# Li-Jinjie/ndp_nmpc_qd

Hardware: AMD Instinct MI355X
Metric: NMPC solves/sec (N=20, 1 RTI iter + downwash MLP) at batch (higher is better)
Workload: dtype f64

## Files before the change

ndp_nmpc_qd_amd/batched.py:

```python
import ctypes as C

import numpy as np

from . import _lib
from .params import downwash_params as DP
from .params import nmpc_params as CP


class NdpError(RuntimeError):
    pass


class BatchedNMPC:
    def __init__(self, batch, N=CP.N_node, disturbance=False, n_rti=1, qp_mode=_lib.QP_AUTO, device=0,
                 dt=CP.th_pred, load_mlp=None, **cfg_overrides):
        self._lib = _lib.load()
        if "ipm_refine" not in cfg_overrides and (7 * int(N) - 3 > 192 or cfg_overrides.get("qp_precision", 0)):
            cfg_overrides = dict(cfg_overrides, ipm_refine=0)
        self.cfg = _lib.default_cfg(batch=int(batch), N=int(N), n_rti=int(n_rti), use_fd=int(bool(disturbance)),
                                    qp_mode=int(qp_mode), device=int(device), dt=float(dt), r_horiz=DP.r_horiz,
                                    **cfg_overrides)
        self.B, self.N = int(batch), int(N)
        self.disturbance = bool(disturbance)
        self._h = C.c_void_p()
        rc = self._lib.ndp_create(C.byref(self.cfg), C.byref(self._h))
        if rc != 0:
            self._h = None
            raise NdpError(f"ndp_create failed ({rc}): {self._lib.ndp_last_error(None).decode()}")
        if load_mlp is None:
            load_mlp = self.disturbance
        if load_mlp:
            self.set_mlp_weights(_lib.load_weights())

    def close(self):
        if getattr(self, "_h", None):
            self._lib.ndp_destroy(self._h)
            self._h = None

    def __del__(self):
        try:
            self.close()
        except Exception:
            pass

    def _check(self, rc, what):
        if rc < 0:
            raise NdpError(f"{what} failed ({rc}): {self._lib.ndp_last_error(self._h).decode()}")
        return rc

    def set_mlp_weights(self, blob):
        blob = np.ascontiguousarray(blob, dtype=np.float32)
        self._check(self._lib.ndp_set_mlp_weights(self._h, _lib.ptr(blob), blob.size), "ndp_set_mlp_weights")
        self._mlp_installed = None

    def reset(self, xr, ur):
        xr = _lib.f64(xr, (self.B, self.N + 1, 10))
        ur = _lib.f64(ur, (self.B, self.N, 4))
        self._check(self._lib.ndp_reset(self._h, _lib.ptr(xr), _lib.ptr(ur)), "ndp_reset")

    def update(self, x0, xr, ur, f=None, other=None, ego_xy=None, raise_on_status=True, full=False):
        x0 = _lib.f64(x0, (self.B, 10))
        xr = _lib.f64(xr, (self.B, self.N + 1, 10))
        ur = _lib.f64(ur, (self.B, self.N, 4))
        u0 = np.empty((self.B, 4), dtype=np.float64)
        if f is not None and other is None and np.asarray(f).dtype == np.float64:
            f64 = _lib.f64(f, (self.B, self.N + 1, 3))
            X = U = st = it = None
            if full:
                X, U = np.empty((self.B, self.N + 1, 10)), np.empty((self.B, self.N, 4))
                st, it = np.empty(self.B, dtype=np.int32), np.empty(self.B, dtype=np.int32)
            rc = self._check(self._lib.ndp_step_ex_f64(self._h, _lib.ptr(x0), _lib.ptr(xr), _lib.ptr(ur), _lib.ptr(f64), _lib.ptr(u0),
                                                       _lib.ptr(X), _lib.ptr(U), _lib.ptr(st), _lib.ptr(it)), "ndp_step_ex_f64")
            if rc != 0 and raise_on_status:
                raise Exception("acados acados_ocp_solver returned status {}. Exiting.".format(rc))
            return (u0, X, U, st, it) if full else u0
        f32 = None if f is None else np.ascontiguousarray(f, dtype=np.float32).reshape(self.B, self.N + 1, 3)
        other = _lib.f64(other, (self.B, self.N + 1, 10))
        ego_xy = _lib.f64(ego_xy, (self.B, 2))
        if full:
            X, U = np.empty((self.B, self.N + 1, 10)), np.empty((self.B, self.N, 4))
            st, it = np.empty(self.B, dtype=np.int32), np.empty(self.B, dtype=np.int32)
            rc = self._check(self._lib.ndp_step_ex(self._h, _lib.ptr(x0), _lib.ptr(xr), _lib.ptr(ur), _lib.ptr(f32),
                                                   _lib.ptr(other), _lib.ptr(ego_xy), _lib.ptr(u0), _lib.ptr(X), _lib.ptr(U),
                                                   _lib.ptr(st), _lib.ptr(it)), "ndp_step_ex")
        else:
            rc = self._check(self._lib.ndp_step(self._h, _lib.ptr(x0), _lib.ptr(xr), _lib.ptr(ur), _lib.ptr(f32),
                                                _lib.ptr(other), _lib.ptr(ego_xy), _lib.ptr(u0)), "ndp_step")
        if rc != 0 and raise_on_status:
            raise Exception("acados acados_ocp_solver returned status {}. Exiting.".format(rc))
        return (u0, X, U, st, it) if full else u0

    def update_begin(self, x0, xr, ur, f=None, other=None, ego_xy=None, want_iterate=False):
        x0 = _lib.f64(x0, (self.B, 10))
        xr = _lib.f64(xr, (self.B, self.N + 1, 10))
        ur = _lib.f64(ur, (self.B, self.N, 4))
        f32 = None if f is None else np.ascontiguousarray(f, dtype=np.float32).reshape(self.B, self.N + 1, 3)
        other = _lib.f64(other, (self.B, self.N + 1, 10))
        ego_xy = _lib.f64(ego_xy, (self.B, 2))
        self._check(self._lib.ndp_step_begin(self._h, _lib.ptr(x0), _lib.ptr(xr), _lib.ptr(ur), _lib.ptr(f32), _lib.ptr(other),
                                             _lib.ptr(ego_xy), 1 if want_iterate else 0), "ndp_step_begin")

    def update_end(self, raise_on_status=True, full=False, out=None):
        u0 = np.empty((self.B, 4), dtype=np.float64) if out is None else out
        st = it = X = U = None
        if full:
            X, U = np.empty((self.B, self.N + 1, 10)), np.empty((self.B, self.N, 4))
            st, it = np.empty(self.B, dtype=np.int32), np.empty(self.B, dtype=np.int32)
        rc = self._check(self._lib.ndp_step_end(self._h, _lib.ptr(u0), _lib.ptr(X), _lib.ptr(U), _lib.ptr(st), _lib.ptr(it)),
                         "ndp_step_end")
        if rc != 0 and raise_on_status:
            raise Exception("acados acados_ocp_solver returned status {}. Exiting.".format(rc))
        return (u0, X, U, st, it) if full else u0

    def update_debug(self, x0, xr, ur, f=None, other=None, ego_xy=None):
        x0, xr, ur = _lib.f64(x0, (1, 10)), _lib.f64(xr, (1, self.N + 1, 10)), _lib.f64(ur, (1, self.N, 4))
        f32 = None if f is None else np.ascontiguousarray(f, dtype=np.float32).reshape(1, self.N + 1, 3)
        other, ego_xy = _lib.f64(other, (1, self.N + 1, 10)), _lib.f64(ego_xy, (1, 2))
        u0 = np.empty((1, 4))
        dump = np.zeros(self._lib.ndp_debug_lds_doubles(self.N))
        self._check(self._lib.ndp_step_debug(self._h, _lib.ptr(x0), _lib.ptr(xr), _lib.ptr(ur), _lib.ptr(f32),
                                             _lib.ptr(other), _lib.ptr(ego_xy), _lib.ptr(u0), _lib.ptr(dump)),
                    "ndp_step_debug")
        return u0, dump

    def downwash(self, other, ego_ref, ego_xy=None):
        other = _lib.f64(other, (self.B, self.N + 1, 10))
        ego_ref = _lib.f64(ego_ref, (self.B, self.N + 1, 10))
        ego_xy = _lib.f64(ego_xy, (self.B, 2))
        f = np.empty((self.B, self.N + 1, 3), dtype=np.float32)
        self._check(self._lib.ndp_downwash(self._h, _lib.ptr(other), _lib.ptr(ego_ref), _lib.ptr(ego_xy), _lib.ptr(f)),
                    "ndp_downwash")
        return f

    def throttle_reset(self):
        self._check(self._lib.ndp_throttle_reset(self._h), "ndp_throttle_reset")

    def throttle_update(self, vz, throttle):
        vz, throttle = _lib.f64(vz, (self.B,)), _lib.f64(throttle, (self.B,))
        k = np.empty(self.B)
        self._check(self._lib.ndp_throttle_update(self._h, _lib.ptr(vz), _lib.ptr(throttle), _lib.ptr(k)), "ndp_throttle_update")
        return k

    def throttle_state(self):
        st = np.empty((self.B, 8))
        self._check(self._lib.ndp_throttle_get_state(self._h, _lib.ptr(st)), "ndp_throttle_get_state")
        return st

    def actuator_cmd(self, u0, k_throttle):
        u0, k = _lib.f64(u0, (self.B, 4)), _lib.f64(k_throttle, (self.B,))
        cmd = np.empty((self.B, 4))
        self._check(self._lib.ndp_actuator_cmd(self._h, _lib.ptr(u0), _lib.ptr(k), _lib.ptr(cmd)), "ndp_actuator_cmd")
        return cmd

    def relay_reset(self):
        self._check(self._lib.ndp_relay_reset(self._h), "ndp_relay_reset")

    def relay_formation(self, form):
        form = _lib.f64(form, (self.B, 3))
        off = np.empty((self.B, 3))
        self._check(self._lib.ndp_relay_formation(self._h, _lib.ptr(form), _lib.ptr(off)), "ndp_relay_formation")
        return off

    def relay_reference(self, xr_lead):
        xr_lead = _lib.f64(xr_lead, (self.B, self.N + 1, 10))
        out = np.empty_like(xr_lead)
        self._check(self._lib.ndp_relay_reference(self._h, _lib.ptr(xr_lead), _lib.ptr(out)), "ndp_relay_reference")
        return out

    def ref_set_trajectory(self, coeff_x, coeff_y, coeff_z, coeff_yaw, time_cum, time_seg, final_pt):
        time_seg = _lib.f64(time_seg)
        n_seg = time_seg.shape[1]
        cx, cy, cz = (_lib.f64(np.reshape(c, (self.B, n_seg * 8)), (self.B, n_seg * 8)) for c in (coeff_x, coeff_y, coeff_z))
        cyaw = _lib.f64(np.reshape(coeff_yaw, (self.B, n_seg * 4)), (self.B, n_seg * 4))
        time_cum, final_pt = _lib.f64(time_cum, (self.B, n_seg + 1)), _lib.f64(final_pt, (self.B, 3))
        self._check(self._lib.ndp_ref_set_trajectory(self._h, n_seg, _lib.ptr(cx), _lib.ptr(cy), _lib.ptr(cz), _lib.ptr(cyaw),
                                                     _lib.ptr(time_cum), _lib.ptr(_lib.f64(time_seg, (self.B, n_seg))),
                                                     _lib.ptr(final_pt)), "ndp_ref_set_trajectory")

    def ref_window(self, t):
        t = _lib.f64(t, (self.B,))
        xr, ur = np.empty((self.B, self.N + 1, 10)), np.empty((self.B, self.N, 4))
        self._check(self._lib.ndp_ref_window(self._h, _lib.ptr(t), _lib.ptr(xr), _lib.ptr(ur)), "ndp_ref_window")
        return xr, ur

    def ref_list_reset(self):
        self._check(self._lib.ndp_ref_list_reset(self._h), "ndp_ref_list_reset")

    def ref_list_fix_pt(self, x_odom, quirk_b1=True):
        x_odom = _lib.f64(x_odom, (self.B, 10))
        self._check(self._lib.ndp_ref_list_fix_pt(self._h, _lib.ptr(x_odom), int(bool(quirk_b1))), "ndp_ref_list_fix_pt")

    def ref_list_window(self, t=None):
        t = _lib.f64(t, (self.B,))
        xr, ur = np.empty((self.B, self.N + 1, 10)), np.empty((self.B, self.N, 4))
        self._check(self._lib.ndp_ref_list_window(self._h, _lib.ptr(t), _lib.ptr(xr), _lib.ptr(ur)), "ndp_ref_list_window")
        return xr, ur

    def ref_list_advance_device(self, t, stream=None):
        import torch
        self._check(self._lib.ndp_ref_list_advance_device(self._h, self._dptr(t, torch.float64, (self.B,)), self._stream(stream)),
                    "ndp_ref_list_advance_device")

    def ref_list_window_device(self, xr_out, ur_out, stream=None):
        import torch
        self._check(self._lib.ndp_ref_list_window_device(
            self._h, self._dptr(xr_out, torch.float64, (self.B, self.N + 1, 10)),
            self._dptr(ur_out, torch.float64, (self.B, self.N, 4)), self._stream(stream)), "ndp_ref_list_window_device")

    def ref_window_device(self, t, xr_out, ur_out, stream=None):
        import torch
        self._check(self._lib.ndp_ref_window_device(
            self._h, self._dptr(t, torch.float64, (self.B,)), self._dptr(xr_out, torch.float64, (self.B, self.N + 1, 10)),
            self._dptr(ur_out, torch.float64, (self.B, self.N, 4)), self._stream(stream)), "ndp_ref_window_device")

    def tick_config(self, other_index=None, gate=True):
        oi = None if other_index is None else np.ascontiguousarray(other_index, dtype=np.int32).reshape(self.B)
        self._check(self._lib.ndp_tick_config(self._h, _lib.ptr(oi), 1 if gate else 0), "ndp_tick_config")

    def tick_reset(self):
        self._check(self._lib.ndp_tick_reset(self._h), "ndp_tick_reset")

    def _tick_in(self, x_odom, t, vz, throttle, estimate, want_u0):
        flags = (_lib.TICK_ESTIMATE if estimate else 0) | (_lib.TICK_WANT_U0 if want_u0 else 0)
        if t is not None and np.ndim(t) == 0:
            t, flags = np.array([float(t)]), flags | _lib.TICK_T_UNIFORM
        else:
            t = _lib.f64(t, (self.B,))
        return (_lib.f64(x_odom, (self.B, 10)), t, _lib.f64(vz, (self.B,)), _lib.f64(throttle, (self.B,)), flags)

    def tick_begin(self, x_odom, t=None, vz=None, throttle=None, estimate=False, want_u0=False):
        x, t, vz, th, flags = self._tick_in(x_odom, t, vz, throttle, estimate, want_u0)
        self._check(self._lib.ndp_tick_begin(self._h, _lib.ptr(x), _lib.ptr(t), _lib.ptr(vz), _lib.ptr(th), flags), "ndp_tick_begin")

    def tick_end(self, raise_on_status=True, full=False, out=None):
        cmd = np.empty((self.B, 4)) if out is None else out
        u0 = st = it = None
        if full:
            u0, st, it = np.empty((self.B, 4)), np.empty(self.B, dtype=np.int32), np.empty(self.B, dtype=np.int32)
        rc = self._check(self._lib.ndp_tick_end(self._h, _lib.ptr(cmd), _lib.ptr(u0), _lib.ptr(st), _lib.ptr(it)), "ndp_tick_end")
        if rc != 0 and raise_on_status:
            raise Exception("acados acados_ocp_solver returned status {}. Exiting.".format(rc))
        return (cmd, u0, st, it) if full else cmd

    def tick(self, x_odom, t=None, vz=None, throttle=None, estimate=False, raise_on_status=True, full=False):
        x, t, vz, th, flags = self._tick_in(x_odom, t, vz, throttle, estimate, full)
        cmd = np.empty((self.B, 4))
        u0 = st = it = None
        if full:
            u0, st, it = np.empty((self.B, 4)), np.empty(self.B, dtype=np.int32), np.empty(self.B, dtype=np.int32)
        rc = self._check(self._lib.ndp_tick(self._h, _lib.ptr(x), _lib.ptr(t), _lib.ptr(vz), _lib.ptr(th), flags, _lib.ptr(cmd),
                                            _lib.ptr(u0), _lib.ptr(st), _lib.ptr(it)), "ndp_tick")
        if rc != 0 and raise_on_status:
            raise Exception("acados acados_ocp_solver returned status {}. Exiting.".format(rc))
        return (cmd, u0, st, it) if full else cmd

    def tick_device(self, x_odom, cmd_out, t=None, vz=None, throttle=None, estimate=False, u0_out=None, stream=None):
        import torch
        B = self.B
        flags = _lib.TICK_ESTIMATE if estimate else 0
        if t is not None and not isinstance(t, torch.Tensor):
            t_host = np.array([float(t)])
            tp, flags = _lib.ptr(t_host), flags | _lib.TICK_T_UNIFORM
        else:
            tp = self._dptr(t, torch.float64, (B,))
        self._check(self._lib.ndp_tick_device(
            self._h, self._dptr(x_odom, torch.float64, (B, 10)), tp,
            self._dptr(vz, torch.float64, (B,)), self._dptr(throttle, torch.float64, (B,)), flags,
            self._dptr(cmd_out, torch.float64, (B, 4)), self._dptr(u0_out, torch.float64, (B, 4)), self._stream(stream)),
            "ndp_tick_device")

    def tick_config_remote(self, windows, other_index, gate=True):
        import torch
        assert isinstance(windows, torch.Tensor) and windows.is_cuda and windows.is_contiguous() and windows.dtype == torch.float64
        assert windows.dim() == 3 and windows.shape[1] == self.N + 1 and windows.shape[2] in (6, 10)
        oi = np.ascontiguousarray(other_index, dtype=np.int32).reshape(self.B)
        self._tick_windows = windows
# ... 552 lines not shown
```

ndp_nmpc_qd_amd/csrc/host.hpp:

```cpp
#pragma once
#include <hip/hip_runtime.h>

#include <atomic>
#include <cstdint>
#include <memory>
#include <mutex>
#include <string>
#include <vector>

#include "wave_gfx950.hpp"
#include "cfg_params.hpp"
#include "kern_args.hpp"
#include "rti_table.hpp"

#define NDP_HIDDEN __attribute__((visibility("hidden")))

using namespace ndp;

struct ndp_handle {
    ndp_cfg cfg;
    RtiParams P;
    int lds_per_wave = 0;
    int waves = 4;
    int n_simd = 1024;
    mutable std::atomic<uint64_t> rti_launched{0};
    bool use_queue = false;
    bool queue_auto = false;
    unsigned long long *hIpm = nullptr;
    unsigned long long ipm_seen = 0, steps_seen = 0;
    unsigned queue_launches = 0;
    hipStream_t stream = nullptr;
    double *dX = nullptr, *dU = nullptr;
    float *dForce = nullptr, *dFrag = nullptr;
    double *dKC = nullptr;
    int *dTables = nullptr;
    signed char *dAct = nullptr;
    int sens_level = 0;
    double *dSensU0 = nullptr, *dSensU = nullptr, *dSensX = nullptr;
    double *dPSensXr = nullptr, *dPSensUr = nullptr, *dPSensF = nullptr;
    double *dVjp = nullptr;
    int *dVjpSt = nullptr;
    signed char *dVjpAct = nullptr;
    float *dFragT = nullptr, *dGwPart = nullptr;
    double *dThr = nullptr;
    double *dStamps = nullptr;
    double *dTraj = nullptr;
    int traj_seg = 0;
    double *dRingX = nullptr, *dRingU = nullptr;
    unsigned long long list_n = 0;
    int segc_par = 0;
    int list_step = 5;
    int *dTickIndex = nullptr;
    double *dTickThrust = nullptr;
    bool tick_gate = true;
    const double *tick_remote = nullptr;
    int tick_remote_stride = 6;
    struct TickSlot { bool busy = false, want_u0 = false; } tslot[2];
    double *dRelay = nullptr;
    double *sThr = nullptr;
    float *dForceAB[2] = {nullptr, nullptr};
    unsigned long long *dProto = nullptr;
    hipStream_t aux = nullptr;
    hipEvent_t evFork = nullptr, evJoin = nullptr;
    unsigned prefetch_timeout_us = 100000, pf_groups_rti = 1, pf_ntiles = 1;
    unsigned *dQctr = nullptr;
    int *dQids = nullptr;
    bool have_mlp = false;
    unsigned char *dIn = nullptr, *dOut = nullptr;
    size_t off_x0 = 0, off_xr = 0, off_ur = 0, off_f = 0, off_other = 0, off_ego = 0, in_bytes = 0;
    size_t off_u0 = 0, off_st = 0, off_it = 0, out_bytes = 0, out_all = 0;
    double *sx0 = nullptr, *sxr = nullptr, *sur = nullptr, *sother = nullptr, *sego = nullptr, *su0 = nullptr, *sdbg = nullptr;
    float *sf = nullptr;
    int *dStatus = nullptr, *dIters = nullptr;
    const int *lastStatus = nullptr, *lastIters = nullptr;
    struct HostSlot {
        unsigned char *hIn = nullptr, *hOut = nullptr;
        hipEvent_t evOut = nullptr;
        bool busy = false, want_iter = false;
        double *dump = nullptr;
    } slot[2];
    bool slots_ready = false;
    bool track_steps = false;
    bool last_step_tracked = false;
    bool track_pending = false;
    hipEvent_t stepDone[4] = {nullptr, nullptr, nullptr, nullptr};
    unsigned step_seq = 0;
    double host_us[4] = {0, 0, 0, 0};
    int host_cores = 0, pack_threads = 0;
    int slot_head = 0, slot_tail = 0, slots_busy = 0;
    std::unique_ptr<struct PackPool> pool;
    hipEvent_t evLast = nullptr;
    bool ev_pending = false;
    int timing = 0;
    int64_t launch_no[2] = {0, 0};
    bool timing_open = false;
    struct Ev { hipEvent_t a, b; int kind; };
    std::vector<Ev> events;
    std::mutex mu;
    std::string err;
};

#define NDP_HIP(h, call)                                                                   \
    do {                                                                                   \
        hipError_t e_ = (call);                                                            \
        if (e_ != hipSuccess) {                                                            \
            (h)->err = std::string(#call) + ": " + hipGetErrorString(e_);                  \
            return -(int)e_ - 1000;                                                        \
        }                                                                                  \
    } while (0)

static inline RingGeom ring_geom(const ndp_handle *h) { return RingGeom{h->list_step, h->cfg.N + 1}; }

enum { FRT_TOTAL = 2 * 128 * 64 };
enum { VJ_MAX_GROUPS = 256 };
static inline int mlp_vjp_groups(const ndp_handle *h)
{
    const int ntiles = (h->cfg.batch * (h->cfg.N + 1) + 31) / 32, ngroups = (ntiles + 3) / 4;
    return ngroups < VJ_MAX_GROUPS ? ngroups : VJ_MAX_GROUPS;
}

enum { TICK_ESTIMATE = NDP_TICK_ESTIMATE, TICK_WANT_U0 = NDP_TICK_WANT_U0, TICK_T_UNIFORM = NDP_TICK_T_UNIFORM };

static inline size_t nxs(const ndp_handle *h) { return (size_t)h->cfg.batch * (h->cfg.N + 1) * NX; }
static inline size_t nus(const ndp_handle *h) { return (size_t)h->cfg.batch * h->cfg.N * NU; }
static inline size_t nfs(const ndp_handle *h) { return (size_t)h->cfg.batch * (h->cfg.N + 1) * 3; }
static inline size_t up256(size_t n) { return (n + 255) & ~(size_t)255; }
static inline size_t act_bytes(const ndp_handle *h) { return (size_t)h->cfg.batch * (size_t)act_pitch(h->cfg.N); }
struct TrajView {
    double *coeff, *tcum, *tseg, *fpt, *segc[2];
    int *hint;
    size_t doubles;
};
static inline TrajView traj_view(double *base, size_t B, size_t S)
{
    TrajView v;
    size_t o = 0;
    auto part = [&](size_t n) { double *p = base ? base + o : nullptr; o += n; return p; };
    v.coeff = part(B * S * 28); v.tcum = part(B * (S + 1)); v.tseg = part(B * S); v.fpt = part(B * 3);
    v.segc[0] = part(B * SEGC_PER); v.hint = reinterpret_cast<int *>(part((B * 4 + 7) / 8)); v.segc[1] = part(B * SEGC_PER);
    v.doubles = o;
    return v;
}
static inline TrajView traj_view(const ndp_handle *h) { return traj_view(h->dTraj, (size_t)h->cfg.batch, (size_t)h->traj_seg); }
static inline void copy_ipm_iters(int32_t *dst, const int32_t *src, size_t n)
{
    for (size_t i = 0; i < n; ++i) dst[i] = src[i] & ITERS_IPM_MASK;
}

struct Neigh {
    const double *other = nullptr;
    int stride = NX;
    const int *index = nullptr;
    const double *ego_xy = nullptr;
    size_t pitch = 0;
    size_t ego_pitch = 0;
};

struct StepOut {
    int *status = nullptr;
    int *iters = nullptr;
    double *Xm = nullptr, *Um = nullptr;
    hipEvent_t done = nullptr;
    size_t xr_pitch = 0, ur_pitch = 0;
    double *cmd = nullptr;
    const double *kthr = nullptr;
    double *thrust_keep = nullptr;
    bool f_f64 = false;
    const TickArgs *tick = nullptr;
};

enum RecomputeId { RC_WVJP, RC_JVP, RC_VJP };

extern "C" {
NDP_HIDDEN bool queue_shape(const ndp_handle *h);
NDP_HIDDEN void launch_kern(const ndp_handle *h, RtiId id, hipStream_t s, KernArgs &ka, SensArgs &sa, hipEvent_t start = nullptr,
                            hipEvent_t stop = nullptr);
NDP_HIDDEN const void *recompute_kernel(RecomputeId id, bool n20);
NDP_HIDDEN hipError_t rti_set_lds(bool sens, int lds_bytes, const char **what);
NDP_HIDDEN hipError_t mlp_prepare(void);
NDP_HIDDEN int launch_mlp(ndp_handle *h, const Neigh &nb, const double *d_ego, float *d_f, hipStream_t s, size_t ego_pitch = 0);
NDP_HIDDEN void launch_tick_pre(const TickPre &a, hipStream_t s);
NDP_HIDDEN int sens_refuse(ndp_handle *h, const char *what);
NDP_HIDDEN int note_stream(ndp_handle *h, hipStream_t s);
NDP_HIDDEN int set_device(ndp_handle *h);
NDP_HIDDEN int wait_all(ndp_handle *h);
NDP_HIDDEN int begin_timing(ndp_handle *h, hipStream_t s, int kind, bool defer = false);
NDP_HIDDEN int end_timing(ndp_handle *h, hipStream_t s);
NDP_HIDDEN bool can_fuse(const ndp_handle *h);
NDP_HIDDEN int launch_rti(ndp_handle *h, const double *d_x0, const double *d_xr, const double *d_ur, const float *d_f, double *d_u0,
                          double *d_dbg, hipStream_t s, const Neigh *nb = nullptr, const StepOut *so = nullptr, bool prefetched = false);
NDP_HIDDEN int enqueue_step(ndp_handle *h, const double *d_x0, const double *d_xr, const double *d_ur, const float *d_f, const Neigh &nb,
                            double *d_u0, double *d_dbg, hipStream_t s, const StepOut *so = nullptr);
NDP_HIDDEN int ensure_slots(ndp_handle *h);
NDP_HIDDEN int launch_plant_force(ndp_handle *h, const double *d_x, const int *d_index, int gate, double scale, double *d_f, double *d_xy,
                                  hipStream_t s);
NDP_HIDDEN hipError_t mlp_multi_prepare(void);
NDP_HIDDEN int check_neigh(ndp_handle *h, const char *who, int K);
NDP_HIDDEN int launch_mlp_multi(ndp_handle *h, const double *d_other, int other_stride, const int *d_index, int K, const double *d_ego,
                                const double *d_ego_xy, float *d_f, hipStream_t s);
NDP_HIDDEN int launch_plant_force_multi(ndp_handle *h, const double *d_x, const int *d_index, int K, int gate, double scale, double *d_f,
                                        double *d_xy, hipStream_t s);
NDP_HIDDEN ThrCfg thr_cfg(const ndp_handle *h);
NDP_HIDDEN RefCfg ref_cfg(const ndp_handle *h, double toff);
NDP_HIDDEN void launch_throttle_reset(const ndp_handle *h);
NDP_HIDDEN int launch_list_window(ndp_handle *h, double *d_xr, double *d_ur, hipStream_t s);
NDP_HIDDEN int ensure_tick(ndp_handle *h);
NDP_HIDDEN int tick_step_enqueue(ndp_handle *h, hipStream_t s, const double *x_odom, double *cmd, double *u0, const double *windows,
                                 unsigned long long pos);
NDP_HIDDEN void make_fragments_t(const float *blob, float *frt);
NDP_HIDDEN hipError_t mlp_vjp_prepare(void);
NDP_HIDDEN int peer_mapped(const void *p);
NDP_HIDDEN void launch_pack_pv_list(const double *base, size_t pitch, int np1, double *pv, size_t B, hipStream_t s);
}
NDP_HIDDEN TickPre tick_pre(const ndp_handle *h, bool adv, const double *t, double t_all, bool est, const double *x_odom, const double *vz,
                            const double *throttle, double *pv = nullptr);

struct Entry {
    ndp_handle *h;
    std::unique_lock<std::mutex> lk;
    hipStream_t s = nullptr;
    int rc = -1;
    Entry(ndp_handle *h_, bool args, void *stream = nullptr, const char *refuse = nullptr) : h(h_)
    {
        if (!h) return;
// ... 15 lines not shown
```

ndp_nmpc_qd_amd/csrc/ndp_hip.hip:

```cpp
#include <hip/hip_runtime.h>
#include <hip/hip_ext.h>

#include <sched.h>
#include <stdio.h>

#include <atomic>
#include <chrono>
#include <condition_variable>
#include <cstdlib>
#include <cstring>
#include <memory>
#include <mutex>
#include <new>
#include <string>
#include <thread>
#include <type_traits>
#include <vector>

#include "host.hpp"
#include "cond_qp.hpp"
#include "mlp_tile.hpp"

namespace ndp {

// ... 154 lines not shown
    for (auto &e : h->events) { (void)hipEventDestroy(e.a); (void)hipEventDestroy(e.b); }
    if (h->evLast) (void)hipEventDestroy(h->evLast);
    if (h->aux) { (void)hipStreamSynchronize(h->aux); (void)hipStreamDestroy(h->aux); }
    for (hipEvent_t e : {h->evFork, h->evJoin, h->stepDone[0], h->stepDone[1], h->stepDone[2], h->stepDone[3]})
        if (e) (void)hipEventDestroy(e);
    h->pool.reset();
    void *ptrs[] = {h->dForceAB[0], h->dForceAB[1], h->dProto, h->dRingX, h->dTraj, h->dTables, h->dStamps, h->dRelay, h->dThr, h->sThr, h->dKC, h->dForce, h->dFrag,
                    h->dIn, h->dOut, h->sdbg, h->dQctr, h->dQids, h->dTickIndex, h->dTickThrust, h->dAct,
                    h->dSensU0, h->dSensU, h->dSensX, h->dPSensXr, h->dPSensUr, h->dPSensF, h->dVjp, h->dVjpSt, h->dVjpAct, h->dFragT, h->dGwPart};
    for (void *p : ptrs)
        if (p) (void)hipFree(p);
    for (auto &sl : h->slot) {
        if (sl.hIn) (void)hipHostFree(sl.hIn);
        if (sl.hOut) (void)hipHostFree(sl.hOut);
        if (sl.evOut) (void)hipEventDestroy(sl.evOut);
    }
    if (h->hIpm) {
        (void)hipDeviceSynchronize();
        (void)hipHostFree(h->hIpm);
    }
    if (h->stream) (void)hipStreamDestroy(h->stream);
    delete h;
    return 0;
}

static bool as_gamma_holds(const ndp_cfg &c, const double *Rd)
{
    if (c.as_iter_max <= 0) return true;
    double rd = 0.0;
    for (int i = 0; i < 4; ++i) rd = std::max(rd, std::fabs(c.dt * Rd[i]));
    return std::isfinite(c.as_gamma) && c.as_gamma >= NDP_AS_GAMMA_FLOOR * rd;
}

int ndp_create(const ndp_cfg *cfg, ndp_handle **out)
{
    if (!cfg || !out) { g_create_err = "ndp_create: null argument"; return -1; }
    *out = nullptr;
    if (cfg->batch < 1 || cfg->N < 2 || slots_for(cfg->N) > 5 || cfg->n_rti < 1 || cfg->qp_precision < 0 || cfg->qp_precision > 6 ||
        cfg->work_queue < 0 || cfg->work_queue > 2 || !(cfg->ts_nmpc > 0.0) || cfg->dt < cfg->ts_nmpc) {
        g_create_err = "ndp_create: need batch >= 1, 2 <= N <= 46, n_rti >= 1, qp_precision in 0..6, work_queue in 0..2, 0 < ts_nmpc <= dt";
        return -2;
    }
    if (cfg->qp_precision >= 5 && (cfg->N % 4 != 0 || cfg->N > 40)) {
        g_create_err = "ndp_create: the condensed study (qp_precision 5 / 6) tiles the 4N x 4N Hessian by 16: N must be a multiple of 4, at most 40";
        return -2;
    }
    if (!as_gamma_holds(*cfg, cfg->Rd)) {
        g_create_err = "ndp_create: as_gamma must be finite and at least 1e8 * max(dt * Rd) when as_iter_max > 0 (a weaker pin does not hold "
                       "its input on the bound)";
        return -2;
    }
    if (cfg->ipm_refine > 0 && (slots_for(cfg->N) > 3 || cfg->qp_precision != 0)) {
        g_create_err = "ndp_create: ipm_refine > 0 is not served for this shape: the refinement path (stiff sweeps + second solves while a STATE bound's "
                       "barrier term exceeds refine_gamma) lives in the three-slot fp64 kernels only (N <= 27, qp_precision 0); the five-slot kernels "
                       "(N >= 28) sit at the register limit without it.  Set ipm_refine = 0: strongly active state bounds at a tight tolerance then "
                       "end in status 4 (never a silent answer)";
        return -2;
    }
    {
        const double ratio = cfg->dt / cfg->ts_nmpc, nearest = (double)(long long)(ratio + 0.5);
        if (ratio - nearest > 1e-9 || nearest - ratio > 1e-9) {
            g_create_err = "ndp_create: dt must be a whole multiple of ts_nmpc (node spacing = every k-th entry of the reference list)";
            return -2;
        }
    }
    int ndev = 0;
    hipError_t e = hipGetDeviceCount(&ndev);
    if (e != hipSuccess || ndev <= cfg->device) {
        g_create_err = std::string("ndp_create: no usable HIP device (") + hipGetErrorString(e) + ")";
        return -3;
    }
    ndp_handle *h = new (std::nothrow) ndp_handle;
    if (!h) return -4;
    h->cfg = *cfg;
    h->P = to_params(*cfg);
    h->list_step = (int)(cfg->dt / cfg->ts_nmpc + 0.5);
    h->lds_per_wave = (lds_doubles(cfg->N) + 1) & ~1;
    if (cfg->qp_precision >= 5) h->lds_per_wave += (cond_extra_doubles(cfg->N) + 1) & ~1;
    const size_t per_wave_bytes = (size_t)h->lds_per_wave * sizeof(double);
    h->waves = 4;
    while (h->waves > 1 && per_wave_bytes * h->waves > 160 * 1024) h->waves >>= 1;
    if (const char *e = getenv("NDP_DEV_WAVES")) {
        const int w = atoi(e);
        if ((w == 1 || w == 2 || w == 4) && w <= h->waves) h->waves = w;
    }
    auto fail = [&](const char *what, hipError_t err) {
        g_create_err = std::string("ndp_create: ") + what + ": " + hipGetErrorString(err);
        ndp_destroy(h);
        return -5;
    };
    if ((e = hipSetDevice(cfg->device)) != hipSuccess) return fail("hipSetDevice", e);
    {
        hipDeviceProp_t prop;
        if ((e = hipGetDeviceProperties(&prop, cfg->device)) != hipSuccess) return fail("hipGetDeviceProperties", e);
        h->n_simd = 4 * prop.multiProcessorCount;
    }
    if (cfg->work_queue == 1 && !(queue_shape(h) && cfg->qp_mode == NDP_QP_AUTO)) {
        g_create_err = "ndp_create: work_queue = 1 needs qp_mode AUTO, qp_precision 0 and (N, n_rti) = (20, 1) or (40, 2)";
        delete h;
        return -2;
    }
    h->queue_auto = cfg->work_queue == 0 && queue_shape(h) && cfg->qp_mode == NDP_QP_AUTO && cfg->N == 20 && cfg->batch >= 2 * h->n_simd;
    h->use_queue = cfg->work_queue == 1 || (cfg->work_queue == 0 && queue_shape(h) && cfg->qp_mode == NDP_QP_AUTO && cfg->N == 40);
    if (h->queue_auto) {
        if ((e = hipHostMalloc((void **)&h->hIpm, 64, hipHostMallocDefault)) != hipSuccess) return fail("hipHostMalloc (work-list counter)", e);
        h->hIpm[0] = h->hIpm[1] = 0;
    }
    if ((e = hipStreamCreateWithFlags(&h->stream, hipStreamNonBlocking)) != hipSuccess) return fail("hipStreamCreate", e);
    if ((e = hipEventCreateWithFlags(&h->evLast, hipEventDisableTiming)) != hipSuccess) return fail("hipEventCreate", e);
    const size_t B = cfg->batch;
#define ALLOC(p, n)                                                                      \
    if ((e = hipMalloc((void **)&(p), (n))) != hipSuccess) return fail("hipMalloc " #p, e)
    ALLOC(h->dForce, nfs(h) * 4); ALLOC(h->dFrag, FR_TOTAL * 4); ALLOC(h->dFragT, FRT_TOTAL * 4); ALLOC(h->dGwPart, (size_t)mlp_vjp_groups(h) * NDP_MLP_NPARAM * 4); ALLOC(h->dKC, KC_HOST * 8);
    ALLOC(h->dThr, B * 8 * 8); ALLOC(h->sThr, B * 11 * 8);
    ALLOC(h->dRelay, B * 4 * 8);
    ALLOC(h->dQctr, 256); ALLOC(h->dQids, B * 4);
    ALLOC(h->dAct, B * (size_t)act_pitch(cfg->N));
    (void)hipMemsetAsync(h->dAct, 0, B * (size_t)act_pitch(cfg->N), h->stream);
    (void)hipMemsetAsync(h->dRelay, 0, B * 4 * 8, h->stream);
    (void)hipMemsetAsync(h->dQctr, 0, 256, h->stream);
    {
        double kc[KC_HOST];
        fill_kc(h->P, kc);
        if ((e = hipMemcpyAsync(h->dKC, kc, sizeof(kc), hipMemcpyHostToDevice, h->stream)) != hipSuccess) return fail("hipMemcpy kc", e);
        ALLOC(h->dTables, TB_WORDS * 4);
        std::vector<int> tb(TB_WORDS);
        fill_tables(cfg->N, tb.data(), (cfg->qp_precision == 3 || cfg->qp_precision == 4) ? 1 : 0);
        if ((e = hipMemcpyAsync(h->dTables, tb.data(), TB_WORDS * 4, hipMemcpyHostToDevice, h->stream)) != hipSuccess) return fail("hipMemcpy tables", e);
        if ((e = hipStreamSynchronize(h->stream)) != hipSuccess) return fail("hipStreamSynchronize", e);
    }
    {
        size_t o = 0;
        h->off_x0 = o; o += up256(B * NX * 8);
        h->off_xr = o; o += up256(nxs(h) * 8);
        h->off_ur = o; o += up256(nus(h) * 8);
        h->off_f = o; o += up256(nfs(h) * 8);
        h->off_other = o; o += up256(nxs(h) * 8);
        h->off_ego = o; o += up256(B * 2 * 8);
        h->in_bytes = o;
        o = 0;
        h->off_u0 = o; o += up256(B * NU * 8);
        h->off_st = o; o += up256(B * 4);
        h->off_it = o; o += up256(B * 4);
        h->out_bytes = o;
        h->out_all = h->out_bytes + (nxs(h) + nus(h)) * 8;
        ALLOC(h->dIn, h->in_bytes);
        ALLOC(h->dOut, h->out_all);
        h->dX = (double *)(h->dOut + h->out_bytes); h->dU = h->dX + nxs(h);
        h->sx0 = (double *)(h->dIn + h->off_x0); h->sxr = (double *)(h->dIn + h->off_xr); h->sur = (double *)(h->dIn + h->off_ur);
        h->sf = (float *)(h->dIn + h->off_f); h->sother = (double *)(h->dIn + h->off_other); h->sego = (double *)(h->dIn + h->off_ego);
        h->su0 = (double *)(h->dOut + h->off_u0); h->dStatus = (int *)(h->dOut + h->off_st); h->dIters = (int *)(h->dOut + h->off_it);
        h->lastStatus = h->dStatus; h->lastIters = h->dIters;
        ALLOC(h->sdbg, (size_t)(lds_doubles(cfg->N) + DBG_EXTRA) * 8);
    }
#undef ALLOC
    (void)hipMemsetAsync(h->dX, 0, nxs(h) * 8, h->stream);
    (void)hipMemsetAsync(h->dU, 0, nus(h) * 8, h->stream);
    (void)hipMemsetAsync(h->dOut, 0, h->out_bytes, h->stream);
    (void)hipMemsetAsync(h->dForce, 0, nfs(h) * 4, h->stream);
    const int lds_bytes = (int)(per_wave_bytes * h->waves);
    if ((e = mlp_prepare()) != hipSuccess) return fail("hipFuncSetAttribute(mlp_kernel)", e);
    if ((e = mlp_vjp_prepare()) != hipSuccess) return fail("hipFuncSetAttribute(mlp_vjp_kernel)", e);
    if ((e = mlp_multi_prepare()) != hipSuccess) return fail("hipFuncSetAttribute(mlp_multi_kernel)", e);
    const char *what = nullptr;
    if ((e = rti_set_lds(false, lds_bytes, &what)) != hipSuccess) return fail(what, e);
    launch_throttle_reset(h);
    if ((e = hipStreamSynchronize(h->stream)) != hipSuccess) return fail("hipStreamSynchronize", e);
    *out = h;
    return 0;
}

int begin_timing(ndp_handle *h, hipStream_t s, int kind, bool defer)
{
    h->timing_open = false;
    if (!h->timing || (h->launch_no[kind]++ % h->timing) != 0) return 0;
    h->timing_open = true;
    ndp_handle::Ev ev; ev.kind = kind;
    NDP_HIP(h, hipEventCreate(&ev.a)); NDP_HIP(h, hipEventCreate(&ev.b));
    if (!defer) NDP_HIP(h, hipEventRecord(ev.a, s));
    h->events.push_back(ev);
    return 0;
}
int end_timing(ndp_handle *h, hipStream_t s)
{
    if (!h->timing_open) return 0;
    NDP_HIP(h, hipEventRecord(h->events.back().b, s));
    return 0;
}

int note_stream(ndp_handle *h, hipStream_t s)
{
    if (s == h->stream) return 0;
    hipStreamCaptureStatus cs = hipStreamCaptureStatusNone;
    if (hipStreamIsCapturing(s, &cs) != hipSuccess || cs != hipStreamCaptureStatusNone) { (void)hipGetLastError(); return 0; }
    NDP_HIP(h, hipEventRecord(h->evLast, s));
    h->ev_pending = true;
    return 0;
}
int wait_all(ndp_handle *h)
{
    NDP_HIP(h, hipStreamSynchronize(h->stream));
    if (h->ev_pending) {
        NDP_HIP(h, hipEventSynchronize(h->evLast));
        h->ev_pending = false;
    }
    if (h->track_pending) {
        if (h->stepDone[h->step_seq & 3]) NDP_HIP(h, hipEventSynchronize(h->stepDone[h->step_seq & 3]));
        h->track_pending = false;
    }
    return 0;
}

int set_device(ndp_handle *h)
{
    NDP_HIP(h, hipSetDevice(h->cfg.device));
    return 0;
}

enum { QP_WINDOW = 8 };
static void queue_policy(ndp_handle *h, hipStream_t s)
{
    if (!h->queue_auto) return;
    const unsigned long long steps_now = ((volatile unsigned long long *)h->hIpm)[1], ipm_now = ((volatile unsigned long long *)h->hIpm)[0];
    if (steps_now >= h->steps_seen + QP_WINDOW && ipm_now >= h->ipm_seen) {
        const double frac = (double)(ipm_now - h->ipm_seen) / ((double)(steps_now - h->steps_seen) * (double)h->cfg.batch);
        if (frac >= 0.04) h->use_queue = true;
        else if (frac <= 0.015) h->use_queue = false;
        h->ipm_seen = ipm_now;
        h->steps_seen = steps_now;
    }
    if (++h->queue_launches < QP_WINDOW) return;
    h->queue_launches = 0;
    if (hipMemcpyAsync(h->hIpm, reinterpret_cast<unsigned long long *>(h->dQctr + 16), 16, hipMemcpyDeviceToHost, s) != hipSuccess) (void)hipGetLastError();
}

static RtiId rti_pick(const ndp_handle *h, bool fused, bool tick, bool prefetched, int phase)
{
    const int N = h->cfg.N, W = h->waves, pr = h->cfg.qp_precision, wi = W == 4 ? 0 : W == 2 ? 1 : 2;
    const bool ref = N == 20 && h->cfg.n_rti == 1;
    if (pr) {
        if (pr >= 3 && N == 40 && h->cfg.n_rti == 2 && W == 2) return pr == 3 ? K40_F32 : K40_BF16;
        return (RtiId)(KPREC1 + pr - 1);
    }
    if (h->sens_level > 0) {
        RtiId id;
        if (phase) id = phase == 2 ? S20_CONS : fused ? S20F_PROD : S20_PROD;
        else if (N == 20 && W == 4) id = fused ? S20F : S20;
        else if (W == 4) id = fused ? SF_4 : S_4;
        else id = fused ? SF_2 : S_2;
        if (!h->dPSensXr) return id;
        switch (id) {
        case S20F_PROD: return P20F_PROD;
        case S20_PROD: return P20_PROD;
        case S20_CONS: return P20_CONS;
        case S20F: return P20F;
        case S20: return P20;
        case SF_4: return PF_4;
        default: return PF_2;
        }
    }
    if (phase == 2) return N == 20 ? K20_CONS : K40_CONS;
    if (phase == 1) {
        if (N != 20) return K40_PROD;
        if (tick) return fused ? K20F_PROD_TICK : K20_PROD_TICK;
        return fused ? K20F_PROD : K20_PROD;
    }
    if (ref && W == 4) {
        if (tick) return fused ? K20F_TICK : K20_TICK;
        return fused ? K20F : prefetched ? K20_LATE : K20;
    }
    if (ref && W == 2) return fused ? K20F_W2 : K20_W2;
    if (N == 40 && h->cfg.n_rti == 2 && W == 2 && !fused) return K40;
    if (fused) return (RtiId)(K3F_4 + wi);
    return (RtiId)((slots_for(N) <= 3 ? K3_4 : K5_4) + wi);
}

int launch_rti(ndp_handle *h, const double *d_x0, const double *d_xr, const double *d_ur, const float *d_f,
               double *d_u0, double *d_dbg, hipStream_t s, const Neigh *nb, const StepOut *so, bool prefetched)
{
    int *d_status = so && so->status ? so->status : h->dStatus, *d_iters = so && so->iters ? so->iters : h->dIters;
    h->lastStatus = d_status; h->lastIters = d_iters;
    BatchPtrs bp{h->dKC, h->dTables, d_x0, d_xr, d_ur, d_f, h->dX, h->dU, d_u0, d_status, d_iters,
                 so ? so->Xm : nullptr, so ? so->Um : nullptr, d_dbg, h->dStamps,
                 so && so->xr_pitch ? so->xr_pitch : (size_t)(h->cfg.N + 1) * NX, so && so->ur_pitch ? so->ur_pitch : (size_t)h->cfg.N * NU, (size_t)NX,
                 so ? so->cmd : nullptr, so ? so->kthr : nullptr, so ? so->thrust_keep : nullptr, h->cfg.mass, so && so->f_f64 ? 1 : 0,
                 h->dAct};
    const bool fused = nb && nb->other;
    MlpArgs ma{fused ? h->dFrag : nullptr, fused ? nb->other : nullptr, fused ? nb->ego_xy : nullptr, h->dForce,
               h->cfg.r_horiz * h->cfg.r_horiz, fused ? nb->stride : NX, fused ? nb->index : nullptr, fused ? peer_mapped(nb->other) : 0,
               fused && nb->pitch ? nb->pitch : (size_t)(h->cfg.N + 1) * (fused ? nb->stride : NX), fused && nb->ego_pitch ? nb->ego_pitch : (size_t)2};
    QueueArgs qa{h->dQctr, h->dQids, reinterpret_cast<unsigned long long *>(h->dQctr + 16)};
    LateArgs la{prefetched ? h->dProto : nullptr, {h->dForceAB[0], h->dForceAB[1]}, h->prefetch_timeout_us,
                h->pf_groups_rti, h->pf_ntiles};
    KernArgs ka{h->P, bp, h->cfg.batch, h->lds_per_wave, ma, qa, la, so && so->tick ? *so->tick : TickArgs{}};
    SensArgs sa{h->dSensU0, h->sens_level >= 2 ? h->dSensU : nullptr, h->sens_level >= 2 ? h->dSensX : nullptr, h->sens_level};
    const bool tick1 = so && so->tick;
    const int pr = h->cfg.qp_precision;
    const bool q = h->use_queue && !d_dbg && !prefetched;
    h->last_step_tracked = false;
    if (h->track_steps) {
        hipStreamCaptureStatus cs = hipStreamCaptureStatusNone;
        if (hipStreamIsCapturing(s, &cs) != hipSuccess) { (void)hipGetLastError(); cs = hipStreamCaptureStatusNone; }
        if (cs != hipStreamCaptureStatusNone) {
            h->err = "tracked control steps (ndp_track_steps) cannot be launched on a stream that is being captured: switch tracking off "
                     "and order the exchange through the stream (ndp_xchg_begin's after_stream)";
            return -15;
        }
    }
    int rc = begin_timing(h, s, 0, true);
    if (rc) return rc;
    const bool ext_timing = h->timing_open && !q && !pr && !(so && so->done) && !h->track_steps;
    if (h->timing_open && !ext_timing) NDP_HIP(h, hipEventRecord(h->events.back().a, s));
    if (pr && fused) { h->err = "qp_precision != 0 supports f / no disturbance only (run ndp_downwash first)"; return -12; }
    hipEvent_t stop = nullptr;
    if (so && so->done) stop = so->done;
    else if (h->track_steps) { stop = h->stepDone[++h->step_seq & 3]; h->last_step_tracked = true; }
    if (h->sens_level > 0 && (prefetched || tick1)) { h->err = "launch_rti: the late-force and tick forms have no sensitivity kernel"; return -2; }
    launch_kern(h, rti_pick(h, fused, tick1, prefetched, q ? 1 : 0), s, ka, sa, ext_timing ? h->events.back().a : nullptr,
                ext_timing ? h->events.back().b : q || pr ? nullptr : stop);
    if (ext_timing) h->timing_open = false;
    NDP_HIP(h, hipGetLastError());
    if (q) {
        KernArgs kc = ka;
        kc.bp.f = fused ? h->dForce : d_f;
        kc.ma.frag = nullptr; kc.ma.other = nullptr;
        if (h->cfg.n_rti == 1 && h->cfg.as_iter_max <= 0) kc.P.qp_mode = QP_IPM_ALWAYS;
        launch_kern(h, rti_pick(h, fused, tick1, prefetched, 2), s, kc, sa);
        NDP_HIP(h, hipGetLastError());
        if (stop) hipExtLaunchKernelGGL(queue_reset_kernel, dim3(1), dim3(64), 0, s, nullptr, stop, 0, h->dQctr, qa.ipm_total);
        else hipLaunchKernelGGL(queue_reset_kernel, dim3(1), dim3(64), 0, s, h->dQctr, qa.ipm_total);
        NDP_HIP(h, hipGetLastError());
    } else if (pr && stop) NDP_HIP(h, hipEventRecord(stop, s));
    const int rce = end_timing(h, s);
    queue_policy(h, s);
    return rce;
}

bool can_fuse(const ndp_handle *h)
{
    return h->cfg.qp_precision == 0 && h->cfg.N + 1 <= 32 && slots_for(h->cfg.N) <= 3 &&
           (size_t)h->lds_per_wave * sizeof(double) * h->waves >= FR_TOTAL * sizeof(float);
}

int enqueue_step(ndp_handle *h, const double *d_x0, const double *d_xr, const double *d_ur, const float *d_f,
                 const Neigh &nb, double *d_u0, double *d_dbg, hipStream_t s, const StepOut *so)
{
    if (h->dPSensXr && !(nb.other && can_fuse(h)) && !(h->cfg.N == 20 && h->waves == 4)) {
        h->err = "ndp_step: parameter sensitivities at N != 20 (or 2 instances per workgroup) need the fused step (neighbour windows "
                 "given): the unfused kernel of a run-time horizon has none";
        return -2;
    }
    if ((d_f || nb.other) && !h->cfg.use_fd) { h->err = "ndp_step: a disturbance force needs use_fd = 1 (NDP model)"; return -8; }
    if (nb.other) {
        if (d_f) { h->err = "ndp_step: pass either f or other, not both"; return -7; }
        if (nb.stride != 10 && nb.stride != 6) { h->err = "ndp_step: other_stride must be 10 or 6"; return -13; }
        if (!h->have_mlp) { h->err = "downwash requested but ndp_set_mlp_weights was never called"; return -6; }
        if (can_fuse(h)) return launch_rti(h, d_x0, d_xr, d_ur, nullptr, d_u0, d_dbg, s, &nb, so);
        int rc = launch_mlp(h, nb, d_xr, h->dForce, s, so ? so->xr_pitch : 0);
        if (rc) return rc;
        d_f = h->dForce;
    }
    return launch_rti(h, d_x0, d_xr, d_ur, d_f, d_u0, d_dbg, s, nullptr, so);
}

int ndp_reset_device(ndp_handle *h, const void *d_xr, const void *d_ur, void *stream)
{
    Entry g(h, d_xr && d_ur, stream);
    if (g.rc) return g.rc;
    NDP_HIP(h, hipMemcpyAsync(h->dX, d_xr, nxs(h) * 8, hipMemcpyDefault, g.s));
    NDP_HIP(h, hipMemcpyAsync(h->dU, d_ur, nus(h) * 8, hipMemcpyDefault, g.s));
    NDP_HIP(h, hipMemsetAsync(h->dAct, 0, act_bytes(h), g.s));
    return g.noted(0);
}

int ndp_reset(ndp_handle *h, const double *xr, const double *ur)
{
    Entry g(h, xr && ur);
    if (g.rc) return g.rc;
    int rc = wait_all(h);
    if (rc) return rc;
    NDP_HIP(h, hipMemcpyAsync(h->dX, xr, nxs(h) * 8, hipMemcpyDefault, h->stream));
    NDP_HIP(h, hipMemcpyAsync(h->dU, ur, nus(h) * 8, hipMemcpyDefault, h->stream));
    NDP_HIP(h, hipMemsetAsync(h->dAct, 0, act_bytes(h), h->stream));
    return g.synced(0);
}

int ndp_step_device_ex(ndp_handle *h, const void *d_x0, const void *d_xr, const void *d_ur, const void *d_f,
                       const void *d_other, int other_stride, const void *d_other_index, const void *d_ego_xy,
                       void *d_u0, void *stream)
{
    Entry g(h, d_x0 && d_xr && d_ur && d_u0, stream);
    if (g.rc) return g.rc;
    Neigh nb;
    nb.other = (const double *)d_other; nb.stride = other_stride; nb.index = (const int *)d_other_index; nb.ego_xy = (const double *)d_ego_xy;
    return g.noted(enqueue_step(h, (const double *)d_x0, (const double *)d_xr, (const double *)d_ur, (const float *)d_f, nb,
                                (double *)d_u0, nullptr, g.s));
}

int ndp_step_device(ndp_handle *h, const void *d_x0, const void *d_xr, const void *d_ur, const void *d_f,
                    const void *d_other, const void *d_ego_xy, void *d_u0, void *stream)
{
    return ndp_step_device_ex(h, d_x0, d_xr, d_ur, d_f, d_other, NX, nullptr, d_ego_xy, d_u0, stream);
}

int ensure_slots(ndp_handle *h)
{
    if (h->slots_ready) return 0;
    for (int i = 0; i < 2; ++i) {
        ndp_handle::HostSlot &sl = h->slot[i];
        if (!sl.hIn) NDP_HIP(h, hipHostMalloc((void **)&sl.hIn, h->in_bytes, hipHostMallocDefault));
        if (!sl.hOut) {
            NDP_HIP(h, hipHostMalloc((void **)&sl.hOut, h->out_all, hipHostMallocDefault));
            memset(sl.hOut, 0, h->out_bytes);
        }
        if (!sl.evOut) NDP_HIP(h, hipEventCreateWithFlags(&sl.evOut, hipEventDisableTiming));
    }
    int nt = 0;
    h->host_cores = usable_cores();
    if (const char *e = getenv("NDP_PACK_THREADS")) nt = atoi(e);
    else if (h->in_bytes > 2 * PACK_CHUNK) nt = (h->host_cores / 2 > 8 ? 8 : h->host_cores / 2) - 1;
    h->pack_threads = nt > 0 ? (nt > 64 ? 64 : nt) : 0;
    h->pool.reset(new (std::nothrow) PackPool(h->pack_threads));
    if (!h->pool) { h->err = "ensure_slots: out of memory"; return -4; }
    h->slots_ready = true;
    return 0;
}

static int step_begin_locked(ndp_handle *h, const double *x0, const double *xr, const double *ur, const float *f,
                             const double *other, const double *ego_xy, bool want_iter, double *dump, bool f_f64 = false)
{
    const size_t B = h->cfg.batch;
    hipStream_t s = h->stream;
    NDP_HIP(h, hipSetDevice(h->cfg.device));
    int rc = ensure_slots(h);
    if (rc) return rc;
    if (h->slots_busy == 2) { h->err = "ndp_step_begin: two steps are already in flight (call ndp_step_end first)"; return -14; }
    if (h->ev_pending && (rc = wait_all(h))) return rc;
    ndp_handle::HostSlot &sl = h->slot[h->slot_head];
    struct Seg { size_t off; const void *src; size_t len; size_t rows, row_len, src_stride; };
    Seg segs[6];
    int ns = 0;
    size_t o = 0;
    auto up256 = [](size_t x) { return (x + 255) & ~(size_t)255; };
    auto add = [&](const void *src, size_t len, size_t rows = 0, size_t row_len = 0, size_t src_stride = 0) {
        segs[ns] = {o, src, len, rows, row_len, src_stride};
        o += up256(len);
        return segs[ns++].off;
    };
    const size_t rows_o = B * (size_t)(h->cfg.N + 1);
    const size_t o_x0 = add(x0, B * NX * 8), o_xr = add(xr, nxs(h) * 8), o_ur = add(ur, nus(h) * 8);
    const size_t o_f = f ? add(f, nfs(h) * (f_f64 ? 8 : 4)) : 0;
    const size_t o_other = other ? add(other, rows_o * 6 * 8, rows_o, 6 * 8, NX * 8) : 0;
    const size_t o_ego = ego_xy ? add(ego_xy, B * 2 * 8) : 0;
    const size_t used = o;
    std::vector<PackJob> jobs;
    for (int i = 0; i < ns; ++i) {
        if (segs[i].rows) {
            const size_t rows_per = PACK_CHUNK / segs[i].src_stride;
            for (size_t r = 0; r < segs[i].rows; r += rows_per) {
                const size_t n = segs[i].rows - r < rows_per ? segs[i].rows - r : rows_per;
                jobs.push_back({sl.hIn + segs[i].off + r * segs[i].row_len, (const unsigned char *)segs[i].src + r * segs[i].src_stride,
                                segs[i].row_len, n, segs[i].src_stride});
            }
            continue;
        }
        for (size_t c = 0; c < segs[i].len; c += PACK_CHUNK) {
            const size_t n = segs[i].len - c < PACK_CHUNK ? segs[i].len - c : PACK_CHUNK;
            jobs.push_back({sl.hIn + segs[i].off + c, (const unsigned char *)segs[i].src + c, n});
        }
    }
    const int nj = (int)jobs.size();
    PackPool &pool = *h->pool;
    const auto tp0 = std::chrono::steady_clock::now();
    pool.post(jobs.data(), nj);
    for (int i = 0; i < nj; ++i) pool.wait_job(i);
    pool.finish();
    const auto tp1 = std::chrono::steady_clock::now();
    const unsigned char *ib = sl.hIn;
    (void)used;
    Neigh nb;
    nb.other = other ? (const double *)(ib + o_other) : nullptr;
    nb.stride = 6;
    nb.ego_xy = ego_xy ? (const double *)(ib + o_ego) : nullptr;
    StepOut so;
    so.status = (int *)(sl.hOut + h->off_st); so.iters = (int *)(sl.hOut + h->off_it);
    if (want_iter) { so.Xm = (double *)(sl.hOut + h->out_bytes); so.Um = so.Xm + nxs(h); }
    so.f_f64 = f_f64;
    const bool ext_done = !dump && h->cfg.qp_precision == 0 && (!other || can_fuse(h)) && !getenv("NDP_HOST_EVENT_RECORD");
    if (ext_done) so.done = sl.evOut;
    rc = enqueue_step(h, (const double *)(ib + o_x0), (const double *)(ib + o_xr), (const double *)(ib + o_ur),
                      f ? (const float *)(ib + o_f) : nullptr, nb, (double *)(sl.hOut + h->off_u0), dump ? h->sdbg : nullptr, s, &so);
    if (rc) return rc;
    if (!ext_done) NDP_HIP(h, hipEventRecord(sl.evOut, s));
    sl.busy = true; sl.want_iter = want_iter; sl.dump = dump;
    h->host_us[0] = std::chrono::duration<double, std::micro>(tp1 - tp0).count();
    h->host_us[1] = std::chrono::duration<double, std::micro>(std::chrono::steady_clock::now() - tp1).count();
    h->slot_head ^= 1;
    ++h->slots_busy;
    return 0;
}

static int step_end_locked(ndp_handle *h, double *u0, double *X_out, double *U_out, int32_t *status_out, int32_t *iters_out)
{
    const size_t B = h->cfg.batch;
    if (h->slots_busy == 0) { h->err = "ndp_step_end: no step in flight (ndp_step_begin first)"; return -14; }
    if (h->tslot[h->slot_tail].busy) { h->err = "ndp_step_end: the oldest call in flight is a tick (ndp_tick_end it)"; return -14; }
    ndp_handle::HostSlot &sl = h->slot[h->slot_tail];
    NDP_HIP(h, hipSetDevice(h->cfg.device));
    if ((X_out || U_out) && !sl.want_iter) { h->err = "ndp_step_end: the iterate was not requested at ndp_step_begin (flags bit 0)"; return -15; }
    const auto tw0 = std::chrono::steady_clock::now();
    hipError_t e = hipErrorNotReady;
    for (int spin = 0; spin < 4000 && e == hipErrorNotReady; ++spin) e = hipEventQuery(sl.evOut);
    if (e == hipErrorNotReady) e = hipEventSynchronize(sl.evOut);
    if (e == hipSuccess && sl.dump)
        e = hipMemcpy(sl.dump, h->sdbg, (size_t)(lds_doubles(h->cfg.N) + DBG_EXTRA) * 8, hipMemcpyDeviceToHost);
    sl.busy = false;
    h->slot_tail ^= 1;
    --h->slots_busy;
    NDP_HIP(h, e);
    const auto tw1 = std::chrono::steady_clock::now();
    const unsigned char *ho = sl.hOut;
    if (u0) memcpy(u0, ho + h->off_u0, B * NU * 8);
    const int32_t *st = (const int32_t *)(ho + h->off_st);
    if (status_out) memcpy(status_out, st, B * 4);
    if (iters_out) copy_ipm_iters(iters_out, reinterpret_cast<const int32_t *>(ho + h->off_it), B);
    if (X_out) memcpy(X_out, ho + h->out_bytes, nxs(h) * 8);
    if (U_out) memcpy(U_out, ho + h->out_bytes + nxs(h) * 8, nus(h) * 8);
    int w = 0;
    for (size_t i = 0; i < B; ++i) w = st[i] > w ? st[i] : w;
    h->host_us[2] = std::chrono::duration<double, std::micro>(tw1 - tw0).count();
    h->host_us[3] = std::chrono::duration<double, std::micro>(std::chrono::steady_clock::now() - tw1).count();
    return w;
}

int ndp_debug_host_info(ndp_handle *h, int32_t *out3)
{
    if (!h || !out3) return -1;
    std::lock_guard<std::mutex> lk(h->mu);
    out3[0] = (int32_t)std::thread::hardware_concurrency();
    out3[1] = h->slots_ready ? h->host_cores : usable_cores();
    out3[2] = h->slots_ready ? h->pack_threads : -1;
    return 0;
}

int ndp_debug_rti_launched(ndp_handle *h, uint64_t *mask, int32_t *out3)
{
    if (!h) return -1;
    if (mask) *mask = h->rti_launched.exchange(0, std::memory_order_relaxed);
    if (out3) {
        out3[0] = RTI_KERNELS;
        out3[1] = h->waves;
        out3[2] = can_fuse(h) ? 1 : 0;
    }
    return 0;
}

int ndp_debug_host_timing(ndp_handle *h, double *out4)
{
    if (!h || !out4) return -1;
    std::lock_guard<std::mutex> lk(h->mu);
    for (int i = 0; i < 4; ++i) out4[i] = h->host_us[i];
    return 0;
}

int ndp_step_begin(ndp_handle *h, const double *x0, const double *xr, const double *ur, const float *f,
                   const double *other, const double *ego_xy, int flags)
{
    if (!h || !x0 || !xr || !ur) return -1;
    std::lock_guard<std::mutex> lk(h->mu);
    return step_begin_locked(h, x0, xr, ur, f, other, ego_xy, (flags & 1) != 0, nullptr);
}

int ndp_step_end(ndp_handle *h, double *u0, double *X_out, double *U_out, int32_t *status_out, int32_t *iters_out)
{
    if (!h || !u0) return -1;
    std::lock_guard<std::mutex> lk(h->mu);
    return step_end_locked(h, u0, X_out, U_out, status_out, iters_out);
}

static int step_host(ndp_handle *h, const double *x0, const double *xr, const double *ur, const float *f,
                     const double *other, const double *ego_xy, double *u0, double *X_out, double *U_out,
                     int32_t *status_out, int32_t *iters_out, double *dump, bool f_f64 = false)
{
    if (!h || !x0 || !xr || !ur || !u0) return -1;
    std::lock_guard<std::mutex> lk(h->mu);
    if (h->slots_busy) { h->err = "ndp_step: steps begun with ndp_step_begin are still in flight (ndp_step_end them first)"; return -14; }
    int rc = step_begin_locked(h, x0, xr, ur, f, other, ego_xy, X_out || U_out, dump, f_f64);
    if (rc) return rc;
    return step_end_locked(h, u0, X_out, U_out, status_out, iters_out);
}

int ndp_step(ndp_handle *h, const double *x0, const double *xr, const double *ur, const float *f,
             const double *other, const double *ego_xy, double *u0)
{
    return step_host(h, x0, xr, ur, f, other, ego_xy, u0, nullptr, nullptr, nullptr, nullptr, nullptr);
}

int ndp_step_ex(ndp_handle *h, const double *x0, const double *xr, const double *ur, const float *f,
                const double *other, const double *ego_xy, double *u0, double *X_out, double *U_out,
                int32_t *status_out, int32_t *iters_out)
{
    return step_host(h, x0, xr, ur, f, other, ego_xy, u0, X_out, U_out, status_out, iters_out, nullptr);
}

int ndp_step_ex_f64(ndp_handle *h, const double *x0, const double *xr, const double *ur, const double *f, double *u0,
                    double *X_out, double *U_out, int32_t *status_out, int32_t *iters_out)
{
    return step_host(h, x0, xr, ur, reinterpret_cast<const float *>(f), nullptr, nullptr, u0, X_out, U_out, status_out, iters_out, nullptr, f != nullptr);
}

int ndp_step_debug(ndp_handle *h, const double *x0, const double *xr, const double *ur, const float *f,
                   const double *other, const double *ego_xy, double *u0, double *lds_dump)
{
    if (h && h->cfg.batch != 1) { h->err = "ndp_step_debug: batch must be 1"; return -9; }
    return step_host(h, x0, xr, ur, f, other, ego_xy, u0, nullptr, nullptr, nullptr, nullptr, lds_dump);
}

int ndp_get_iterate(ndp_handle *h, double *X, double *U)
{
    Entry g(h, true);
    if (g.rc) return g.rc;
    int rc = wait_all(h);
    if (rc) return rc;
    if (X) NDP_HIP(h, hipMemcpy(X, h->dX, nxs(h) * 8, hipMemcpyDefault));
    if (U) NDP_HIP(h, hipMemcpy(U, h->dU, nus(h) * 8, hipMemcpyDefault));
    return 0;
}

int ndp_set_iterate(ndp_handle *h, const double *X, const double *U)
{
    Entry g(h, true);
    if (g.rc) return g.rc;
    int rc = wait_all(h);
    if (rc) return rc;
    if (X) NDP_HIP(h, hipMemcpy(h->dX, X, nxs(h) * 8, hipMemcpyDefault));
    if (U) NDP_HIP(h, hipMemcpy(h->dU, U, nus(h) * 8, hipMemcpyDefault));
    NDP_HIP(h, hipMemset(h->dAct, 0, act_bytes(h)));
    return 0;
}

int ndp_get_active_set(ndp_handle *h, int32_t *sweeps, int8_t *act)
{
    Entry g(h, true);
    if (g.rc) return g.rc;
    int rc = wait_all(h);
    if (rc) return rc;
    const size_t B = (size_t)h->cfg.batch;
    if (sweeps) {
        NDP_HIP(h, hipMemcpy(sweeps, h->lastIters, B * 4, hipMemcpyDefault));
        for (size_t i = 0; i < B; ++i) sweeps[i] = (int32_t)((uint32_t)sweeps[i] >> ITERS_SWEEP_SHIFT);
    }
    if (act) NDP_HIP(h, hipMemcpy(act, h->dAct, act_bytes(h), hipMemcpyDefault));
    return 0;
}

int ndp_set_active_set(ndp_handle *h, const int8_t *act)
{
    Entry g(h, act);
    if (g.rc) return g.rc;
    int rc = wait_all(h);
    if (rc) return rc;
    const size_t n = act_bytes(h);
    for (size_t i = 0; i < n; ++i)
        if (act[i] < -1 || act[i] > 1) { h->err = "ndp_set_active_set: entries are -1, 0 or +1"; return -1; }
    NDP_HIP(h, hipMemcpy(h->dAct, act, n, hipMemcpyDefault));
    return 0;
}

int ndp_get_status(ndp_handle *h, int32_t *status, int32_t *ipm_iters)
{
    Entry g(h, true);
    if (g.rc) return g.rc;
    int rc = wait_all(h);
    if (rc) return rc;
    if (status) NDP_HIP(h, hipMemcpy(status, h->lastStatus, (size_t)h->cfg.batch * 4, hipMemcpyDefault));
    if (ipm_iters) {
        NDP_HIP(h, hipMemcpy(ipm_iters, h->lastIters, (size_t)h->cfg.batch * 4, hipMemcpyDefault));
        copy_ipm_iters(ipm_iters, ipm_iters, (size_t)h->cfg.batch);
    }
    return 0;
}

int ndp_debug_stamps(ndp_handle *h, int enable, double *out)
{
    if (!h) return -1;
    std::lock_guard<std::mutex> lk(h->mu);
    NDP_HIP(h, hipSetDevice(h->cfg.device));
    NDP_HIP(h, hipStreamSynchronize(h->stream));
    NDP_HIP(h, hipDeviceSynchronize());
    const size_t bytes = (size_t)h->cfg.batch * NDP_NSTAMP * 8;
    if (out && h->dStamps) NDP_HIP(h, hipMemcpy(out, h->dStamps, bytes, hipMemcpyDeviceToHost));
    if (enable && !h->dStamps) {
        NDP_HIP(h, hipMalloc((void **)&h->dStamps, bytes));
        NDP_HIP(h, hipMemset(h->dStamps, 0, bytes));
    } else if (!enable && h->dStamps) {
        (void)hipFree(h->dStamps);
        h->dStamps = nullptr;
    }
    return 0;
}

void *ndp_device_iterate_x(ndp_handle *h) { return h ? h->dX : nullptr; }
void *ndp_device_iterate_u(ndp_handle *h) { return h ? h->dU : nullptr; }
void *ndp_device_force(ndp_handle *h) { return h ? h->dForce : nullptr; }
int ndp_work_queue_enabled(ndp_handle *h) { return h ? (int)h->use_queue : -1; }

static int nan_buffer(ndp_handle *h, double *&p, size_t n)
{
    if (p) return 0;
    NDP_HIP(h, hipMalloc((void **)&p, n * 8));
    NDP_HIP(h, hipMemsetAsync(p, 0xff, n * 8, h->stream));
    return 0;
}
static void drop_buffer(double *&p) { if (p) (void)hipFree(p); p = nullptr; }
static int copy_out(ndp_handle *h, double *dst, const double *src, size_t n)
{
    if (dst) NDP_HIP(h, hipMemcpy(dst, src, n * 8, hipMemcpyDeviceToHost));
    return 0;
}

int ndp_sens_enable(ndp_handle *h, int level)
{
    if (!h) return -1;
    std::lock_guard<std::mutex> lk(h->mu);
    if (level < 0 || level > 2) { h->err = "ndp_sens_enable: level must be 0 (off), 1 (du0/dx0) or 2 (also dU/dx0 and dX/dx0)"; return -2; }
    if (level > 0) {
        if (slots_for(h->cfg.N) > 3) { h->err = "ndp_sens_enable: sensitivities are served for N <= 27 only (the five-slot kernels of N >= 28 have none)"; return -2; }
        if (h->cfg.qp_precision != 0) { h->err = "ndp_sens_enable: sensitivities need qp_precision 0 (the fp64 product path)"; return -2; }
        if (h->cfg.n_rti != 1) { h->err = "ndp_sens_enable: sensitivities need n_rti = 1 (the derivative of the step's one QP)"; return -2; }
        if (h->waves != 4 && h->waves != 2) { h->err = "ndp_sens_enable: the sensitivity kernels run 2 or 4 instances per workgroup"; return -2; }
    }
    NDP_HIP(h, hipSetDevice(h->cfg.device));
    int rc = wait_all(h);
    if (rc) return rc;
    const size_t B = h->cfg.batch, N = h->cfg.N;
    const size_t n0 = B * (size_t)sens_u0_pitch(), nu = B * (size_t)sens_u_pitch((int)N), nx = B * (size_t)sens_x_pitch((int)N);
    if (level < 2) { drop_buffer(h->dSensU); drop_buffer(h->dSensX); }
    if (level == 0) { for (double **p : {&h->dSensU0, &h->dPSensXr, &h->dPSensUr, &h->dPSensF}) drop_buffer(*p); h->sens_level = 0; return 0; }
    if ((rc = nan_buffer(h, h->dSensU0, n0))) return rc;
    if (level == 2 && ((rc = nan_buffer(h, h->dSensU, nu)) || (rc = nan_buffer(h, h->dSensX, nx)))) return rc;
    const char *what = nullptr;
    NDP_HIP(h, rti_set_lds(true, (int)((size_t)h->lds_per_wave * sizeof(double) * h->waves), &what));
    NDP_HIP(h, hipStreamSynchronize(h->stream));
    h->sens_level = level;
    return 0;
}

int ndp_sens_level(ndp_handle *h) { return h ? h->sens_level : -1; }

int ndp_get_sens(ndp_handle *h, double *du0_dx0, double *dU_dx0, double *dX_dx0)
{
    if (!h) return -1;
    std::lock_guard<std::mutex> lk(h->mu);
    if (h->sens_level < 1) { h->err = "ndp_get_sens: sensitivities are not enabled (ndp_sens_enable)"; return -2; }
    if ((dU_dx0 || dX_dx0) && h->sens_level < 2) { h->err = "ndp_get_sens: dU/dx0 and dX/dx0 need sensitivity level 2"; return -2; }
    NDP_HIP(h, hipSetDevice(h->cfg.device));
    int rc = wait_all(h);
    if (rc) return rc;
    const size_t B = h->cfg.batch;
    if ((rc = copy_out(h, du0_dx0, h->dSensU0, B * sens_u0_pitch()))) return rc;
    if ((rc = copy_out(h, dU_dx0, h->dSensU, B * sens_u_pitch(h->cfg.N)))) return rc;
    return copy_out(h, dX_dx0, h->dSensX, B * sens_x_pitch(h->cfg.N));
}

void *ndp_device_sens_u0(ndp_handle *h) { return h ? h->dSensU0 : nullptr; }
void *ndp_device_sens_u(ndp_handle *h) { return h ? h->dSensU : nullptr; }
void *ndp_device_sens_x(ndp_handle *h) { return h ? h->dSensX : nullptr; }
// ... 222 lines not shown
```

ndp_nmpc_qd_amd/csrc/rti_kernels.hip:

```cpp
#include <hip/hip_runtime.h>
#include <hip/hip_ext.h>

#include <type_traits>

#include "wave_gfx950.hpp"
#include "cfg_params.hpp"
#include "cond_qp.hpp"
#include "host.hpp"
#include "mlp_common.hpp"
#include "mlp_tile.hpp"
#include "ref_point.hpp"
#include "tick_wave.hpp"

namespace ndp {

__device__ __forceinline__ void bind_instance(RtiIo &io, const BatchPtrs &bp, int inst, int N)
{
    const size_t nx = (size_t)(N + 1) * NX, nu = (size_t)N * NU, nf = (size_t)(N + 1) * 3;
    io.x0 = bp.x0 + (size_t)inst * bp.x0_pitch;
    io.xr = bp.xr + inst * bp.xr_pitch;
    io.ur = bp.ur + inst * bp.ur_pitch;
    io.f = bp.f ? bp.f + inst * nf * (bp.f_f64 ? 2 : 1) : nullptr;
    io.f_is_f64 = bp.f_f64;
    io.X = bp.X + inst * nx;
    io.U = bp.U + inst * nu;
    io.Xm = bp.Xm ? bp.Xm + inst * nx : nullptr;
    io.Um = bp.Xm ? bp.Um + inst * nu : nullptr;
    io.u0 = bp.u0 + (size_t)inst * NU;
    io.status = bp.status + inst;
    io.iters = bp.iters + inst;
    io.dbg = bp.dbg;
    io.f_in_lds = 0;
    io.kc = bp.kc;
    io.tables = bp.tables;
    io.stamps = bp.stamps ? bp.stamps + (size_t)inst * NDP_NSTAMP : nullptr;
    io.act = bp.act ? bp.act + (size_t)inst * act_pitch(N) : nullptr;
    if (NDP_RARELY(bp.cmd != nullptr)) {
        io.cmd = bp.cmd + (size_t)inst * NU;
        io.thrust_keep = bp.thrust_keep + inst;
        io.kthr = bp.kthr[inst];
        io.cmd_mass = bp.cmd_mass;
    }
}

#ifndef NDP_RTI_ATTR
#define NDP_RTI_ATTR
#endif
template <int NSLOT, int WAVES, bool FUSED, int NC = 0, int PREC = 0, int NRC = (NC ? 1 : 0), int QMODE = 0, bool TICK = false>
__global__ __launch_bounds__(64 * WAVES) NDP_RTI_ATTR void rti_kernel(KernArgs ka)
{
    constexpr bool SENS = false, PSENS = false;
    const SensArgs sa{};
    const PSensArgs pa{};
    extern __shared__ __attribute__((aligned(16))) double smem[];
    __shared__ unsigned wg_done;
#include "rti_kernel_body.inc"
}

template <int WAVES, bool FUSED, int NC, int QMODE>
__global__ __launch_bounds__(64 * WAVES) void rti_sens_kernel(KernArgs ka, SensArgs sa)
{
    constexpr int NSLOT = 3, PREC = 0, NRC = NC ? 1 : 0;
    constexpr bool TICK = false, SENS = true, PSENS = false;
    const PSensArgs pa{};
    extern __shared__ __attribute__((aligned(16))) double smem[];
    __shared__ unsigned wg_done;
#include "rti_kernel_body.inc"
}

template <int WAVES, bool FUSED, int NC, int QMODE>
__global__ __launch_bounds__(64 * WAVES) void rti_psens_kernel(KernArgs ka, SensArgs sa, PSensArgs pa)
{
    constexpr int NSLOT = 3, PREC = 0, NRC = NC ? 1 : 0;
    constexpr bool TICK = false, SENS = true, PSENS = true;
    extern __shared__ __attribute__((aligned(16))) double smem[];
    __shared__ unsigned wg_done;
#include "rti_kernel_body.inc"
}

#define NDP_RECOMPUTE_PROLOGUE                                                                     \
    extern __shared__ __attribute__((aligned(16))) double smem[];                                  \
    const RtiParams &P = ka.P;                                                                     \
    const int waves = (int)(blockDim.x >> 6), wave = (int)(threadIdx.x >> 6);                      \
    const int inst = __builtin_amdgcn_readfirstlane((int)blockIdx.x * waves + wave);               \
    if (inst >= ka.B) return;                                                                      \
    const int N = NC ? NC : P.N;                                                                   \
    RtiIo io;                                                                                      \
    bind_instance(io, ka.bp, inst, N);                                                             \
    const int lpw = NC ? ((lds_doubles(NC) + 1) & ~1) : ka.lds_per_wave;                           \
    WaveGfx950::lds_ptr lds = (WaveGfx950::lds_ptr)(smem + (size_t)wave * lpw);                    \
    using Prog = RtiWave<WaveGfx950, 3, NC, true, NC ? 1 : 0>;

template <int NC>
__global__ __launch_bounds__(256) void rti_vjp_kernel(KernArgs ka, VjpArgs va)
{
    NDP_RECOMPUTE_PROLOGUE
    const size_t i = (size_t)inst, nx = (size_t)(N + 1) * NX, nu = (size_t)N * NU, nf = (size_t)(N + 1) * 3;
    const VjpIo vo{va.gu0 ? va.gu0 + i * NU : nullptr, va.gX ? va.gX + i * nx : nullptr, va.gU ? va.gU + i * nu : nullptr,
                   va.gx0 ? va.gx0 + i * NX : nullptr, va.gxr ? va.gxr + i * nx : nullptr, va.gur ? va.gur + i * nu : nullptr,
                   va.gf ? va.gf + i * nf : nullptr};
    typename Prog::InBuf inb;
    double x0v;
    Prog::issue_first(P, io, inb, x0v);
    Prog::template run<false, true, false, false, true>(P, io, lds, inb, x0v, nullptr, nullptr, &vo);
}

template <int NC>
__global__ __launch_bounds__(256) void rti_wvjp_kernel(KernArgs ka, VjpArgs va, double *gmodel)
{
    NDP_RECOMPUTE_PROLOGUE
    const size_t i = (size_t)inst, nx = (size_t)(N + 1) * NX, nu = (size_t)N * NU, nf = (size_t)(N + 1) * 3;
    const VjpIo vo{va.gu0 ? va.gu0 + i * NU : nullptr, va.gX ? va.gX + i * nx : nullptr, va.gU ? va.gU + i * nu : nullptr,
                   va.gx0 ? va.gx0 + i * NX : nullptr, va.gxr ? va.gxr + i * nx : nullptr, va.gur ? va.gur + i * nu : nullptr,
                   va.gf ? va.gf + i * nf : nullptr};
    typename Prog::InBuf inb;
    double x0v;
    Prog::issue_first(P, io, inb, x0v);
    Prog::template run<false, true, false, false, true, true>(P, io, lds, inb, x0v, nullptr, nullptr, &vo, gmodel + i * 16);
}

template <int NC>
__global__ __launch_bounds__(256) void rti_jvp_kernel(KernArgs ka, JvpArgs ja)
{
    NDP_RECOMPUTE_PROLOGUE
    const size_t i = (size_t)inst * (size_t)ja.T, nx = (size_t)(N + 1) * NX, nu = (size_t)N * NU, nf = (size_t)(N + 1) * 3;
    const JvpIo jo{ja.tx0 ? ja.tx0 + i * NX : nullptr, ja.txr ? ja.txr + i * nx : nullptr, ja.tur ? ja.tur + i * nu : nullptr,
                   ja.tf ? ja.tf + i * nf : nullptr, ja.du0 ? ja.du0 + i * NU : nullptr, ja.dX ? ja.dX + i * nx : nullptr,
                   ja.dU ? ja.dU + i * nu : nullptr, ja.T};
    typename Prog::InBuf inb;
    double x0v;
    Prog::issue_first(P, io, inb, x0v);
    Prog::template run<false, true, false, false, false, false, true>(P, io, lds, inb, x0v, nullptr, nullptr, nullptr, nullptr, &jo);
}

#undef NDP_RECOMPUTE_PROLOGUE

__global__ void mfma_probe_kernel(const double *a, const double *b, const double *c, double *d)
{
    const int l = (int)threadIdx.x;
    WaveGfx950::vd4 acc;
    for (int r = 0; r < 4; ++r) acc.r[r] = c[r * 64 + l];
    acc = WaveGfx950::mfma(a[l], b[l], acc);
    for (int r = 0; r < 4; ++r) d[r * 64 + l] = acc.r[r];
    d[256 + l] = WaveGfx950::readlane(a[l], 37) + WaveGfx950::wave_sum(b[l]) + WaveGfx950::wave_min(a[l]) + WaveGfx950::wave_max(a[l]);
    d[320 + l] = WaveGfx950::mfma4(a[l], b[l], c[l]);
    d[384 + l] = WaveGfx950::rowb<0>(a[l]);
    d[448 + l] = WaveGfx950::rowb<1>(a[l]);
    d[512 + l] = WaveGfx950::rowb<2>(a[l]);
    d[576 + l] = WaveGfx950::rowb<3>(a[l]);
    d[640 + l] = WaveGfx950::rowror4<1>(a[l]);
    d[704 + l] = WaveGfx950::rowror4<2>(a[l]);
    d[768 + l] = WaveGfx950::rowror4<3>(a[l]);
}

__global__ void mfma_probe32_kernel(const float *a, const float *b, const float *c, float *d, int mode)
{
    const int l = (int)threadIdx.x;
    WaveGfx950F32::md4 acc;
    for (int r = 0; r < 4; ++r) acc.r[r] = c[r * 64 + l];
    if (mode == 0) acc = WaveGfx950F32::mfma(a[l], b[l], acc);
    else {
        float av[4], bv[4];
        for (int i = 0; i < 4; ++i) { av[i] = a[i * 64 + l]; bv[i] = b[i * 64 + l]; }
        acc = WaveGfx950BF16::mfma_k(av, bv, 4, acc);
    }
    for (int r = 0; r < 4; ++r) d[r * 64 + l] = acc.r[r];
    double x = (double)a[l];
    x = x + WaveGfx950F32::csum1(x);
    x = x + WaveGfx950F32::csum2(x);
    d[256 + l] = (float)x;
}

__global__ __launch_bounds__(256) void mlp_kernel(const float *__restrict__ fr, const double *__restrict__ other,
                                                  const double *__restrict__ ego, const double *__restrict__ ego_xy,
                                                  float *__restrict__ fout, int rows, int np1, double r2,
                                                  int other_stride, const int *__restrict__ other_index, int other_sys,
                                                  size_t other_pitch, size_t ego_pitch, size_t ego_xy_pitch)
{
    extern __shared__ __attribute__((aligned(16))) float wsm[];
    const int lane = (int)(threadIdx.x & 63u), wave = (int)(threadIdx.x >> 6);
    const int j = lane & 31, h = lane >> 5;
    const int ntiles = (rows + 31) / 32;
    const int tile = (int)blockIdx.x * 4 + wave;
    lds_f32 wl = (lds_f32)wsm;
// ... 220 lines not shown
```

ndp_nmpc_qd_amd/csrc/rti_wave.hpp:

```cpp
#pragma once
#define NDP_RARELY(x) (__builtin_expect_with_probability(!!(x), 0, 0.9999))

#ifndef NDP_D
#define NDP_D inline
#endif
#if defined(__clang__)
#define NDP_UNROLL_STAGES _Pragma("unroll UNROLL_STAGES")
#define NDP_UNROLL_SWEEP _Pragma("unroll UNROLL_SWEEP")
#define NDP_KEEP_LOOP _Pragma("unroll 1")
#else
#define NDP_UNROLL_STAGES
#define NDP_UNROLL_SWEEP
#define NDP_KEEP_LOOP
#endif
#ifdef NDP_FINE_STAMPS
#define NDP_FINE(x) x
#else
#define NDP_FINE(x)
#endif
#ifndef NDP_HD
#define NDP_HD inline
#endif

namespace ndp {

enum { NX = 10, NU = 4 };
enum { QP_AUTO = 0, QP_IPM_ALWAYS = 1 };
enum { MB_STRIDE = 138, CB_STRIDE = 48 };
enum { MB_PV = 0, MB_Q = 48, MB_B = 76, MB_ZERO = 86, MB_ONE = 87, MB_H = 88, MB_KT = 89, MB_DUMP = 137 };
enum { CB_QQ = 0, CB_QE = 16, CB_RE = 26, CB_DEX = 30, CB_ZERO = 36, CB_QBV = 37, CB_DEU = 40, CB_RB = 44 };
enum { KC_ZERO = 0, KC_ONE = 1, KC_H = 2, KC_QD = 3, KC_RD = 13, KC_LBV = 17, KC_UBV = 21, KC_LBU = 24, KC_UBU = 28, KC_SC = 32, KC_DUMP = 48,
       KC_LBVM = 50, KC_UBVM = 53, KC_LBUM = 56, KC_UBUM = 60, KC_SIZE = 64, KC_HOST = 64 };
static_assert(CB_RE - CB_DEU == (CB_QE + 3) - (CB_DEX + 3), "gradient entry: the same distance from the diagonal entry for u and v bounds");
static_assert(CB_RB - CB_DEU == CB_QBV - (CB_DEX + 3), "base gradient: the same distance from the diagonal entry for u and v bounds");
static_assert(KC_UBU - KC_LBU == KC_UBV - KC_LBV, "upper bound: the same distance from the lower bound for u and v bounds");
static_assert(KC_RD - KC_LBU == (KC_QD + 3) - KC_LBV, "weight: the same distance from the lower bound for u and v bounds");
enum { SL_GE = CB_RE - CB_DEU, SL_GB = CB_RB - CB_DEU, SL_UB = KC_UBU - KC_LBU, SL_DW = KC_RD - KC_LBU };

struct RtiParams {
    int N, n_rti, use_fd, qp_mode, iter_max;
    double dt, inv_mass, g;
    double Qd[10], Rd[4], lbu[4], ubu[4], lbv[3], ubv[3];
    double mu0, thr0, tol, tau, auto_margin, mu_floor;
    int refine;
    double refine_gamma;
    int as_iter_max;
    double as_gamma;
    double h_6, h2_6, h4_24, h3_6, h4_12, two_over_h2, inv2m;
};

NDP_HD void fill_quotients(RtiParams &p)
{
    const double h = p.dt, h2 = h * h;
    p.h_6 = h / 6.0; p.h2_6 = h2 / 6.0; p.h4_24 = h2 * h2 / 24.0; p.h3_6 = h * h2 / 6.0; p.h4_12 = h2 * h2 / 12.0;
    p.two_over_h2 = 2.0 / h2;
    p.inv2m = 1.0 / (2.0 * (7 * p.N - 3));
}

enum { NDP_NSTAMP = 24 };

struct RtiIo {
    const double *x0;
    const double *xr;
    const double *ur;
    const float *f;
    double *X, *U;
    double *u0;
    int *status, *iters;
    double *dbg;
    int f_in_lds;
    const double *kc;
    double *stamps = nullptr;
    const int *tables = nullptr;
    double *Xm = nullptr, *Um = nullptr;
    const float *f_late = nullptr;
    const unsigned long long *late_flag = nullptr, *late_flag2 = nullptr;
    unsigned long long late_want = 0;
    int late_ready = 0;
    unsigned late_timeout_us = 0;
    int *late_missed = nullptr;
    unsigned long long *ipm_ctr = nullptr;
    int *late_slow = nullptr;
    unsigned *late_cnt = nullptr;
    unsigned long long *late_done_word = nullptr;
    unsigned late_gsize = 1;
    void *late_group = nullptr;
    unsigned late_group_size = 1;
    double *cmd = nullptr, *thrust_keep = nullptr;
    double kthr = 0.0, cmd_mass = 0.0;
    int have_xrN = 0;
    double xrN[10] = {0, 0, 0, 0, 0, 0, 0, 0, 0, 0};
    int f_is_f64 = 0;
    signed char *act = nullptr;
};
NDP_HD int act_pitch(int N) { return 4 * N; }

struct SensIo {
    double *du0, *dU, *dX;
    int level;
};
NDP_HD int sens_u0_pitch() { return NU * NX; }
NDP_HD int sens_u_pitch(int N) { return N * NU * NX; }
NDP_HD int sens_x_pitch(int N) { return (N + 1) * NX * NX; }
struct PSensIo {
    double *dxr, *dur, *df;
};
NDP_HD int psens_xr_pitch(int N) { return NU * (N + 1) * NX; }
NDP_HD int psens_ur_pitch(int N) { return NU * N * NU; }
NDP_HD int psens_f_pitch(int N) { return NU * (N + 1) * 3; }
struct VjpIo {
    const double *gu0, *gX, *gU;
    double *gx0, *gxr, *gur, *gf;
};
struct JvpIo {
    const double *tx0, *txr, *tur, *tf;
    double *du0, *dX, *dU;
    int T;
};
enum { ITERS_SWEEP_SHIFT = 16, ITERS_IPM_MASK = 0xffff, COND_ACCEPTED = 0x1000 };
constexpr double COND_STAT_MAX = 0.3;

struct LdsMap {
    int KC, SC, XI, UI, ZX, ZU, CX, CU, ZD, MB, CB, KT, TXR, TUR, TF, AS, total;
};

NDP_HD LdsMap make_map(int N)
{
    LdsMap m;
    int o = 0;
    m.KC = o; o += KC_SIZE;
    m.SC = m.KC + KC_SC;
    m.XI = o; o += (N + 1) * NX;
    m.UI = o; o += N * NU;
    m.ZX = o; o += (N + 1) * NX;
    m.ZU = o; o += N * NU;
    m.CX = o; o += (N + 1) * NX;
    m.CU = o; o += N * NU;
    m.ZD = o; o += (N + 1) * NX + N * NU;
    m.MB = o; o += N * MB_STRIDE;
    m.CB = o; o += (N + 1) * CB_STRIDE;
    m.AS = o; o += N * NU;
    m.total = o;
    m.KT = m.MB + MB_KT;
    m.TXR = m.ZX;
    m.TUR = m.TXR + (N + 1) * NX;
    m.TF = m.TUR + N * NU;
    return m;
}

NDP_HD int lds_doubles(int N) { return make_map(N).total; }
enum { DBG_EXTRA = 32 };
NDP_HD void lds_layout(int N, int *out)
{
    const LdsMap m = make_map(N);
    out[0] = m.XI; out[1] = m.MB; out[2] = m.CB; out[3] = MB_STRIDE; out[4] = CB_STRIDE; out[5] = m.total; out[6] = m.total; out[7] = 0;
}

NDP_HD void fill_kc(const RtiParams &P, double *kc)
{
    for (int i = 0; i < KC_HOST; ++i) kc[i] = 0.0;
    kc[KC_ONE] = 1.0;
    kc[KC_H] = P.dt;
    for (int i = 0; i < 10; ++i) kc[KC_QD + i] = P.Qd[i];
    for (int i = 0; i < 4; ++i) { kc[KC_RD + i] = P.Rd[i]; kc[KC_LBU + i] = P.lbu[i]; kc[KC_UBU + i] = P.ubu[i]; }
    for (int i = 0; i < 3; ++i) { kc[KC_LBV + i] = P.lbv[i]; kc[KC_UBV + i] = P.ubv[i]; }
    const double um = (P.qp_mode == QP_AUTO && P.as_iter_max > 0) ? 0.0 : P.auto_margin;
    for (int i = 0; i < 4; ++i) { kc[KC_LBUM + i] = P.lbu[i] + um; kc[KC_UBUM + i] = P.ubu[i] - um; }
    for (int i = 0; i < 3; ++i) { kc[KC_LBVM + i] = P.lbv[i] + P.auto_margin; kc[KC_UBVM + i] = P.ubv[i] - P.auto_margin; }
}

template <class W, int NSLOT, int NC = 0, bool HT = false, int NR = 0, int PREC = 0, bool LEAN = false, int COND = 0>
struct RtiWave {
    static NDP_D int horizon(const RtiParams &P) { return NC ? NC : P.N; }
    static constexpr int UNROLL_STAGES = NC > 0 ? NC : 1;
    static constexpr int RESYM = 10;
    using vd = typename W::vd;
    using vi = typename W::vi;
    using vb = typename W::vb;
    using vd4 = typename W::vd4;
    using md = typename W::md;
    using md4 = typename W::md4;
    static constexpr bool MMA4 = W::has_mma4 && PREC == 0;
#ifndef NDP_DELTA_MAX_N
#define NDP_DELTA_MAX_N 40
#endif
    static constexpr int DELTA_MAX_N = NDP_DELTA_MAX_N;
    static NDP_D md mma4(md a, md b, md c) { return W::mfma4(a, b, c); }
    static NDP_D md4 mma(md a, md b, const md4 &c)
    {
        if constexpr (W::packed_k) {
            const md aa[1] = {a}, bb[1] = {b};
            return W::mfma_k(aa, bb, 1, c);
        } else if constexpr (PREC == 0) {
            return W::mfma(a, b, c);
        } else {
            md4 d = W::mfma(W::round_op(a, PREC), W::round_op(b, PREC), c);
            for (int r = 0; r < 4; ++r) d.r[r] = W::round_op(d.r[r], 1);
            return d;
        }
    }
    template <int n>
    static NDP_D md4 mman(const md *a, const md *b, const md4 &c)
    {
        if constexpr (W::packed_k) return W::mfma_k(a, b, n, c);
        else {
            md4 d = c;
            for (int i = 0; i < n; ++i) d = mma(a[i], b[i], d);
            return d;
        }
    }
    static NDP_D vi lane_it() { if constexpr (NR == 1) return W::lane(); else return W::lane_here(); }
    static constexpr bool PACKL = MMA4;
    static constexpr int linv_regs(int n) { return PACKL ? (n + 3) / 4 : n; }
    template <class F>
    static NDP_D void linv_reg(md *linv, int q, F &&f)
    {
        switch (q) {
#define NDP_LC(i) case i: f(linv[i]); break;
        NDP_LC(0) NDP_LC(1) NDP_LC(2) NDP_LC(3) NDP_LC(4) NDP_LC(5) NDP_LC(6) NDP_LC(7)
        NDP_LC(8) NDP_LC(9) NDP_LC(10) NDP_LC(11) NDP_LC(12) NDP_LC(13) NDP_LC(14) NDP_LC(15)
#undef NDP_LC
        default: break;
        }
    }
    static_assert(NC <= 64, "linv_reg serves packs of up to 16 registers");
    static NDP_D void linv_put(md *linv, int k, int N, md v)
    {
        if constexpr (PACKL) {
            const bool whole = (k & 3) == 3 || k == N - 1;
            const vb mine = ((W::lane() >> 2) & 3) == (k & 3);
            linv_reg(linv, k >> 2, [&](md &r) { r = whole ? v : W::msel(mine, v, r); });
        } else linv[k] = v;
    }
    static NDP_D md linv_get(const md *linv, int k)
    {
        if constexpr (PACKL) {
            md v = W::to_m(vd(0.0));
            linv_reg(const_cast<md *>(linv), k >> 2, [&](md &r) { v = r; });
            switch (k & 3) {
            case 0: return W::template rowror4<3>(v);
            case 1: return W::template rowror4<2>(v);
            case 2: return W::template rowror4<1>(v);
            default: return v;
            }
        } else return linv[k];
    }
    static NDP_D int mb(int k) { return k * int(MB_STRIDE); }
    static NDP_D int cb(int k) { return k * int(CB_STRIDE); }
    using lp = typename W::lds_ptr;

    struct Tables {
        vi mk_off[3];
        vi fw_off[3];
        vi mu_off;
        vi c_off[4];
        vi kt_off[3];
        vi kt_st[3];
        vi zu_st, zx_st[3];
        vi kt_st4;
        vi zx_st4;
        vb kt_pred;
        vb lo4;
        vb col0;
        vi lam_w_off;
        vi minor_one[3], minor_pair[3];
        vi own_off;
        vd cof_sign;
        vd adj_a, adj_b;
        vb lam_diag;
    };

    struct Slots {
        vb valid[NSLOT];
        vi zoff[NSLOT];
        vi de_off[NSLOT];
        vi lb_off[NSLOT];
        int io;
        vd lo[NSLOT], hi[NSLOT];
        vd tl[NSLOT], tu[NSLOT], ll[NSLOT], lu[NSLOT];
        vd pl[NSLOT], pu[NSLOT];
    };

    static NDP_HD vi m_entry(const LdsMap &m, vi r, vi c)
    {
        vb isP = r < 3, isPV = r < 6, isQ = (r >= 6) && (r < 10);
        vb colq = (c >= 6) && (c < 10), colu = c >= 12;
        vi colpos = W::sel(colq, c - 6, c - 8);
        vb var_pv = isPV && (colq || colu);
        vb var_q = isQ && (colq || (colu && (c < 15)));
        vb var_b = (r < 10) && (c == 10);
        vb one = (isPV && (c == r)) || ((r == 10) && (c == 10));
        vb hh = isP && (c == r + 3);
        vi rel = W::sel(var_pv, r * 8 + colpos + int(MB_PV),
                 W::sel(var_q, (r - 6) * 7 + colpos + int(MB_Q),
                 W::sel(var_b, r + int(MB_B),
                 W::sel(one, vi(int(MB_ONE)), W::sel(hh, vi(int(MB_H)), vi(int(MB_ZERO)))))));
        return rel + m.MB;
    }

    static NDP_HD vi c_entry(const LdsMap &m, vi row, vi col)
    {
        vb rx = row < 10, cx = col < 10, ru = row >= 12, cu = col >= 12;
        vb dgx = rx && (row == col) && (row < 6);
        vb qq = (row >= 6) && rx && (col >= 6) && cx;
        vb gx = (rx && (col == 10)) || ((row == 10) && cx);
        vi gxi = W::sel(rx, row, col);
        vb dgu = ru && (col == row);
        vb gu = (ru && (col == 10)) || ((row == 10) && cu);
        vi gui = W::sel(ru, row - 12, col - 12);
        vi rel = W::sel(dgx, row + int(CB_DEX),
                 W::sel(qq, (row - 6) * 4 + (col - 6) + int(CB_QQ),
                 W::sel(gx, gxi + int(CB_QE),
                 W::sel(dgu, row - 12 + int(CB_DEU),
                 W::sel(gu, gui + int(CB_RE), vi(int(CB_ZERO)))))));
        return rel + m.CB;
    }

    static NDP_HD void lane_preds(Tables &T)
    {
        vi lane = W::lane();
        vi g = lane >> 4, j = W::lcol(lane), jc = j & 3;
        T.kt_pred = j >= 12;
        T.lo4 = j < 4;
        T.col0 = j == 0;
        T.cof_sign = W::sel(((g + jc) & 1) == 1, vd(-1.0), vd(1.0));
        T.lam_diag = g == jc;
        T.adj_a = MMA4 ? T.cof_sign : W::sel(T.lo4, T.cof_sign, vd(0.0));
        T.adj_b = MMA4 ? -T.cof_sign : W::sel(T.kt_pred, -T.cof_sign, vd(0.0));
    }

    static NDP_HD void build_tables(const LdsMap &m, Tables &T)
    {
        lane_preds(T);
        vi lane = W::lane();
        vi g = lane >> 4, j = W::lcol(lane);
        for (int c = 0; c < 3; ++c) T.mk_off[c] = m_entry(m, g + 4 * c, j);
        for (int r = 0; r < 4; ++r) T.c_off[r] = c_entry(m, g + 4 * r, j);
        for (int c = 0; c < 3; ++c) {
            T.kt_off[c] = (g + 4 * c) * 4 + (j & 3) + m.KT;
            T.fw_off[c] = W::sel(T.kt_pred, T.kt_off[c], m_entry(m, j, g + 4 * c));
            T.kt_st[c] = W::sel(T.kt_pred, T.kt_off[c], vi(m.MB + int(MB_DUMP)));
            vi xi = W::sel(g + 4 * c < 10, g + 4 * c, vi(0));
            T.zx_st[c] = xi + W::sel(T.col0 && (g + 4 * c < 10), vi(m.ZX), vi(m.ZD));
        }
        T.mu_off = m_entry(m, j, g + 12);
        T.zu_st = g + W::sel(T.col0, vi(m.ZU), vi(m.ZD + (m.ZU - m.ZX)));
        vi jc = j & 3;
        T.lam_w_off = W::sel(T.kt_pred, g * 4 + jc + m.SC, vi(m.KC + KC_DUMP));
        for (int a = 0; a < 3; ++a) {
            vi ra = W::sel(g <= a, vi(a + 1), vi(a));
            vi single = W::sel(jc < 2, W::sel(jc == 0, vi(1), vi(0)), W::sel(jc == 2, vi(3), vi(2)));
            vi pair0 = W::sel(jc < 2, vi(2), vi(0));
            T.minor_one[a] = ra * 4 + single + m.SC;
            T.minor_pair[a] = ra * 4 + pair0 + m.SC;
        }
        T.own_off = g * 4 + jc + m.SC;
        vi x4 = ((lane >> 2) & 3) * 4 + g, j4 = lane & 3;
        T.kt_st4 = W::sel(x4 < 12, x4 * 4 + j4 + m.KT, vi(m.MB + int(MB_DUMP)));
        T.zx_st4 = W::sel(x4 < 10, x4, vi(0)) + W::sel((j4 == 0) && (x4 < 10), vi(m.ZX), vi(m.ZD));
    }

    enum { TB_FIELDS = 36 };
    template <class F>
    static NDP_HD void for_each_int(Tables &T, F &&f)
    {
        int i = 0;
        for (int c = 0; c < 3; ++c) { f(i++, T.mk_off[c]); f(i++, T.fw_off[c]); f(i++, T.kt_off[c]); f(i++, T.zx_st[c]); }
        for (int c = 0; c < 3; ++c) f(i++, T.kt_st[c]);
        i++;
        for (int r = 0; r < 4; ++r) f(i++, T.c_off[r]);
        f(i++, T.mu_off); f(i++, T.zu_st); f(i++, T.lam_w_off); f(i++, T.own_off);
        for (int a = 0; a < 3; ++a) f(i++, T.minor_one[a]);
        for (int a = 0; a < 3; ++a) f(i++, T.minor_pair[a]);
        i += 3;
        f(i++, T.kt_st4); f(i++, T.zx_st4);
    }
    static NDP_HD int tb_word(int field, int lane) { return ((field >> 2) * 64 + lane) * 4 + (field & 3); }

    static NDP_D void load_tables(const int *g, Tables &T)
    {
        lane_preds(T);
        vi lane = W::lane();
        for_each_int(T, [&](int i, vi &fld) { fld = W::gldi(g, lane * 4 + ((i >> 2) * 256 + (i & 3))); });
    }

    static constexpr int NMAXS = (64 * NSLOT + 3) / 7;
    static constexpr int RX = ((NMAXS + 1) * NX + 63) / 64, RU = (NMAXS * NU + 63) / 64, RF = ((NMAXS + 1) * 3 + 63) / 64;

    struct InBuf { vd xr[RX], xi[RX], ur[RU], ui[RU], f[RF], kc; };

    static NDP_D void issue_inputs(const RtiParams &P, const RtiIo &io, InBuf &b, bool first)
    {
        const int N = horizon(P);
        vi lane = lane_it();
        const int nx = (N + 1) * NX, nu = N * NU, nf = (N + 1) * 3;
        const bool have_f = P.use_fd && io.f && !io.f_in_lds;
        for (int t = 0; t < RX; ++t) {
            vi i = W::imin(lane + 64 * t, nx - 1);
            b.xr[t] = W::gldu(io.xr, i);
            b.xi[t] = first ? W::gldu(io.X, i) : vd(0.0);
        }
        for (int t = 0; t < RU; ++t) {
            vi i = W::imin(lane + 64 * t, nu - 1);
            b.ur[t] = W::gldu(io.ur, i);
            b.ui[t] = first ? W::gldu(io.U, i) : vd(0.0);
        }
        for (int t = 0; t < RF; ++t) {
            vi i = W::imin(lane + 64 * t, nf - 1);
            b.f[t] = have_f ? (NDP_RARELY(io.f_is_f64 != 0) ? W::gldu(reinterpret_cast<const double *>(io.f), i) : W::gldfu(io.f, i)) : vd(0.0);
        }
        b.kc = first ? W::gldu(io.kc, W::imin(lane, KC_HOST - 1)) : vd(0.0);
    }

    static NDP_D void commit_inputs(const RtiParams &P, const LdsMap &m, const InBuf &b, lp lds, bool first, const RtiIo &io)
    {
        const int N = horizon(P);
        vi lane = lane_it();
        const int nx = (N + 1) * NX, nu = N * NU, nf = (N + 1) * 3;
        for (int t = 0; t < RX; ++t) {
            vi i = W::imin(lane + 64 * t, nx - 1);
            W::st(lds, i + m.TXR, b.xr[t]);
            if (first) W::st(lds, i + m.XI, b.xi[t]);
        }
        if (NDP_RARELY(io.have_xrN != 0)) {
            vd v = vd(io.xrN[9]);
            for (int i = 8; i >= 0; --i) v = W::sel(lane == i, vd(io.xrN[i]), v);
            W::stp(lds, lane + (m.TXR + N * int(NX)), v, lane < int(NX));
        }
        for (int t = 0; t < RU; ++t) {
            vi i = W::imin(lane + 64 * t, nu - 1);
            W::st(lds, i + m.TUR, b.ur[t]);
            if (first) W::st(lds, i + m.UI, b.ui[t]);
        }
        for (int t = 0; t < RF; ++t) {
            vi i = W::imin(lane + 64 * t, nf - 1);
            W::st(lds, i + m.TF, b.f[t]);
        }
        if (first) W::st(lds, W::imin(lane, KC_HOST - 1) + m.KC, b.kc);
        W::sync();
    }

    static NDP_D void build_cost(const RtiParams &P, const LdsMap &m, lp lds)
    {
        const int N = horizon(P);
        vi lane = lane_it();
        constexpr int RA = (4 * (NMAXS + 1) + 63) / 64, RB = (6 * (NMAXS + 1) + 63) / 64, RC = (4 * NMAXS + 63) / 64;
        vd qr[RA][4], qi[RA][4];
        vd xb[RB], rb[RB], wb[RB], uc[RC], rc[RC], wc[RC];
        for (int t = 0; t < RA; ++t) {
            vi task = W::imin(lane + 64 * t, 4 * (N + 1) - 1);
            vi k = task >> 2;
            for (int i = 0; i < 4; ++i) {
                qr[t][i] = W::ld(lds, k * NX + (m.TXR + 6 + i));
                qi[t][i] = W::ld(lds, k * NX + (m.XI + 6 + i));
            }
        }
        for (int t = 0; t < RB; ++t) {
            vi task = W::imin(lane + 64 * t, 6 * (N + 1) - 1);
            vi k = W::div6(task);
            vi i = task - k * 6;
            wb[t] = W::ld(lds, i + (m.KC + KC_QD));
            xb[t] = W::ld(lds, k * NX + i + m.XI);
            rb[t] = W::ld(lds, k * NX + i + m.TXR);
        }
        for (int t = 0; t < RC; ++t) {
            vi ti = W::imin(lane + 64 * t, 4 * N - 1);
            wc[t] = W::ld(lds, (ti & 3) + (m.KC + KC_RD));
            uc[t] = W::ld(lds, ti + m.UI);
            rc[t] = W::ld(lds, ti + m.TUR);
        }
        for (int t = 0; t < RA; ++t) {
            vi task = W::imin(lane + 64 * t, 4 * (N + 1) - 1);
            vi k = task >> 2;
            vi a = task & 3;
            vd s = W::sel(k < N, vd(P.dt), vd(1.0));
            const vd qwr = qr[t][0], qxr = qr[t][1], qyr = qr[t][2], qzr = qr[t][3];
            vd E0[4] = {-qxr, qwr, -qzr, qyr};
            vd E1[4] = {-qyr, qzr, qwr, -qxr};
            vd E2[4] = {-qzr, -qyr, qxr, qwr};
            vd ea0 = W::sel(a == 0, E0[0], W::sel(a == 1, E0[1], W::sel(a == 2, E0[2], E0[3])));
            vd ea1 = W::sel(a == 0, E1[0], W::sel(a == 1, E1[1], W::sel(a == 2, E1[2], E1[3])));
            vd ea2 = W::sel(a == 0, E2[0], W::sel(a == 1, E2[1], W::sel(a == 2, E2[2], E2[3])));
            vd w0 = ea0 * (s * P.Qd[7]), w1 = ea1 * (s * P.Qd[8]), w2 = ea2 * (s * P.Qd[9]);
            vd grad = 0.0;
            vi cb = k * int(CB_STRIDE) + m.CB;
            for (int b = 0; b < 4; ++b) {
                vd h = w0 * E0[b] + w1 * E1[b] + w2 * E2[b];
                W::st(lds, cb + a * 4 + (int(CB_QQ) + b), h);
                grad = grad + h * qi[t][b];
            }
            W::st(lds, cb + a + (int(CB_QE) + 6), grad);
            W::st(lds, cb + int(CB_ZERO), vd(0.0));
        }
        for (int t = 0; t < RB; ++t) {
            vi task = W::imin(lane + 64 * t, 6 * (N + 1) - 1);
            vi k = W::div6(task);
            vi i = task - k * 6;
            vd s = W::sel(k < N, vd(P.dt), vd(1.0));
            vd de = s * wb[t];
            vd grad = de * (xb[t] - rb[t]);
            vi cb = k * int(CB_STRIDE) + m.CB;
            W::st(lds, cb + i + int(CB_DEX), de);
            W::st(lds, cb + i + int(CB_QE), grad);
            W::stp(lds, cb + i + (int(CB_QBV) - 3), grad, i >= 3);
        }
        for (int t = 0; t < RC; ++t) {
            vi task = W::imin(lane + 64 * t, 4 * N - 1);
            vi k = task >> 2;
            vi i = task & 3;
            vd de = P.dt * wc[t];
            vd grad = de * (uc[t] - rc[t]);
            vi cb = k * int(CB_STRIDE) + m.CB;
            W::st(lds, cb + i + int(CB_DEU), de);
            W::st(lds, cb + i + int(CB_RE), grad);
            W::st(lds, cb + i + int(CB_RB), grad);
        }
    }

    static NDP_D void qdot(const vd q[4], const vd w[3], vd o[4])
    {
        o[0] = (-w[0] * q[1] - w[1] * q[2] - w[2] * q[3]) * 0.5;
        o[1] = (w[0] * q[0] + w[2] * q[2] - w[1] * q[3]) * 0.5;
        o[2] = (w[1] * q[0] - w[2] * q[1] + w[0] * q[3]) * 0.5;
        o[3] = (w[2] * q[0] + w[1] * q[1] - w[0] * q[2]) * 0.5;
    }
    static NDP_D void thrust_dir(const vd q[4], vd o[3])
    {
        o[0] = (q[1] * q[3] + q[0] * q[2]) * 2.0;
        o[1] = (q[2] * q[3] - q[0] * q[1]) * 2.0;
        o[2] = 1.0 - (q[1] * q[1] + q[2] * q[2]) * 2.0;
    }
    static NDP_D void thrust_dir_tan(const vd q[4], const vd s[4], vd o[3])
    {
        o[0] = (s[1] * q[3] + q[1] * s[3] + s[0] * q[2] + q[0] * s[2]) * 2.0;
        o[1] = (s[2] * q[3] + q[2] * s[3] - s[0] * q[1] - q[0] * s[1]) * 2.0;
        o[2] = (q[1] * s[1] + q[2] * s[2]) * -4.0;
    }

    struct RkScal {
        vd a3, a4, b4, A, B;
        vd Sv_aa, Sv_ab, Sv_bb, Sp_aa, Sp_ab, Sp_bb;
    };
    static NDP_D void rk_scalars(const RtiParams &P, vd sg, RkScal &K)
    {
        const double h = P.dt, h2 = h * h, hh = 0.5 * h, h6 = P.h_6, hp = P.h2_6;
        K.a3 = 1.0 - sg * (0.25 * h2);
        K.a4 = 1.0 - sg * (0.5 * h2);
        K.b4 = K.a3 * h;
        K.A = 1.0 - sg * (0.5 * h2) + sg * sg * P.h4_24;
        K.B = h - sg * P.h3_6;
        K.Sv_aa = (3.0 + K.a3 * K.a3 * 2.0 + K.a4 * K.a4) * h6;
        K.Sv_ab = (2.0 * hh + K.a3 * (2.0 * hh) + K.a4 * K.b4) * h6;
        K.Sv_bb = (4.0 * hh * hh + K.b4 * K.b4) * h6;
        K.Sp_aa = (2.0 + K.a3 * K.a3) * hp;
        K.Sp_ab = (hh + K.a3 * hh) * hp;
        K.Sp_bb = (2.0 * hh * hh) * hp;
    }

    static NDP_D void linearize(const RtiParams &P, const LdsMap &m, lp lds)
    {
        const int N = horizon(P);
        const double h = P.dt, h2 = h * h, hh = 0.5 * h, h6 = P.h_6, hp = P.h2_6;
        vi lane = lane_it();
        for (int t = 0; t < 4 * N; t += 64) {
            vi task = W::imin(lane + t, 4 * N - 1);
            vi k = task >> 2;
            vi j = task & 3;
            vi xi = k * NX + m.XI + 6, ui = k * NU + m.UI;
            vd q[4] = {W::ld(lds, xi), W::ld(lds, xi + 1), W::ld(lds, xi + 2), W::ld(lds, xi + 3)};
            vd w[3] = {W::ld(lds, ui), W::ld(lds, ui + 1), W::ld(lds, ui + 2)};
            vd c = W::ld(lds, ui + 3);
            vd r[4], e[4], z[4];
            qdot(q, w, r);
            RkScal K;
            rk_scalars(P, (w[0] * w[0] + w[1] * w[1] + w[2] * w[2]) * 0.25, K);
            for (int i = 0; i < 4; ++i) e[i] = W::sel(j == i, vd(1.0), vd(0.0));
            qdot(e, w, z);
            vd Uv[4], Vv[4], Up[4], Vp[4], t1[3], t2[3];
            for (int i = 0; i < 4; ++i) {
                Uv[i] = e[i] * K.Sv_aa + z[i] * K.Sv_ab; Vv[i] = e[i] * K.Sv_ab + z[i] * K.Sv_bb;
                Up[i] = e[i] * K.Sp_aa + z[i] * K.Sp_ab; Vp[i] = e[i] * K.Sp_ab + z[i] * K.Sp_bb;
            }
            vi mb = k * int(MB_STRIDE) + m.MB + j;
            thrust_dir_tan(q, Uv, t1); thrust_dir_tan(r, Vv, t2);
            for (int i = 0; i < 3; ++i) W::st(lds, mb + (int(MB_PV) + (3 + i) * 8), (t1[i] + t2[i]) * c);
            thrust_dir_tan(q, Up, t1); thrust_dir_tan(r, Vp, t2);
            for (int i = 0; i < 3; ++i) W::st(lds, mb + (int(MB_PV) + i * 8), (t1[i] + t2[i]) * c);
            for (int i = 0; i < 4; ++i) W::st(lds, mb + (int(MB_Q) + i * 7), e[i] * K.A + z[i] * K.B);
        }
        for (int t = 0; t < 3 * N; t += 64) {
            vi task = W::imin(lane + t, 3 * N - 1);
            vi k = W::div3(task);
            vi mm = task - k * 3;
            vi xi = k * NX + m.XI + 6, ui = k * NU + m.UI;
            vd q[4] = {W::ld(lds, xi), W::ld(lds, xi + 1), W::ld(lds, xi + 2), W::ld(lds, xi + 3)};
            vd w[3] = {W::ld(lds, ui), W::ld(lds, ui + 1), W::ld(lds, ui + 2)};
            vd c = W::ld(lds, ui + 3);
            vd r[4], em[3], g[4];
            qdot(q, w, r);
            RkScal K;
            rk_scalars(P, (w[0] * w[0] + w[1] * w[1] + w[2] * w[2]) * 0.25, K);
            for (int i = 0; i < 3; ++i) em[i] = W::sel(mm == i, vd(1.0), vd(0.0));
            qdot(q, em, g);
            vd eps = (em[0] * w[0] + em[1] * w[1] + em[2] * w[2]) * 0.5;
            const double da3 = -0.25 * h2, da4 = -0.5 * h2, db4 = -0.25 * h * h2;
            vd Sv_aad = (K.a3 * (2.0 * da3) + K.a4 * da4) * h6, Sv_abd = (K.a4 * db4) * h6;
            vd Sv_bad = (K.b4 * da4 + 2.0 * hh * da3) * h6, Sv_bbd = (K.b4 * db4) * h6;
            vd Sp_aad = K.a3 * (da3 * hp);
            const double Sp_bad = hh * da3 * hp;
            vd dA = sg_lin(P, K), dB = vd(-P.h3_6);
            vd Uv[4], Vv[4], Up[4], Vp[4], t1[3], t2[3];
            for (int i = 0; i < 4; ++i) {
                Uv[i] = (q[i] * Sv_aad + r[i] * Sv_abd) * eps + g[i] * K.Sv_ab;
                Vv[i] = (q[i] * Sv_bad + r[i] * Sv_bbd) * eps + g[i] * K.Sv_bb;
                Up[i] = (q[i] * Sp_aad) * eps + g[i] * K.Sp_ab;
                Vp[i] = (q[i] * Sp_bad) * eps + g[i] * K.Sp_bb;
            }
            vi mb = k * int(MB_STRIDE) + m.MB + 4 + mm;
            thrust_dir_tan(q, Uv, t1); thrust_dir_tan(r, Vv, t2);
            for (int i = 0; i < 3; ++i) W::st(lds, mb + (int(MB_PV) + (3 + i) * 8), (t1[i] + t2[i]) * c);
            thrust_dir_tan(q, Up, t1); thrust_dir_tan(r, Vp, t2);
            for (int i = 0; i < 3; ++i) W::st(lds, mb + (int(MB_PV) + i * 8), (t1[i] + t2[i]) * c);
            for (int i = 0; i < 4; ++i) W::st(lds, mb + (int(MB_Q) + i * 7), (q[i] * dA + r[i] * dB) * eps + g[i] * K.B);
        }
        for (int t = 0; t < N; t += 64) {
            vi k = W::imin(lane + t, N - 1);
            {
                vi mc = k * int(MB_STRIDE) + m.MB;
                W::st(lds, mc + int(MB_ZERO), vd(0.0));
                W::st(lds, mc + int(MB_ONE), vd(1.0));
                W::st(lds, mc + int(MB_H), vd(P.dt));
            }
            vi xi = k * NX + m.XI, ui = k * NU + m.UI, fi = k * 3 + m.TF;
            vd x[10];
            for (int i = 0; i < 10; ++i) x[i] = W::ld(lds, xi + i);
            vd w[3] = {W::ld(lds, ui), W::ld(lds, ui + 1), W::ld(lds, ui + 2)};
            vd c = W::ld(lds, ui + 3);
            vd acc[3] = {W::ld(lds, fi) * P.inv_mass, W::ld(lds, fi + 1) * P.inv_mass, W::ld(lds, fi + 2) * P.inv_mass - P.g};
            vd xn1[10];
            for (int i = 0; i < 10; ++i) xn1[i] = W::ld(lds, xi + (NX + i));
            vd q[4] = {x[6], x[7], x[8], x[9]}, r[4];
            qdot(q, w, r);
            RkScal K;
            rk_scalars(P, (w[0] * w[0] + w[1] * w[1] + w[2] * w[2]) * 0.25, K);
            vd tqq[3], tqr[3], trr[3];
            thrust_dir_tan(q, q, tqq); thrust_dir_tan(q, r, tqr); thrust_dir_tan(r, r, trr);
            vi mb = k * int(MB_STRIDE) + m.MB;
            for (int i = 0; i < 3; ++i) {
                const double e3 = i == 2 ? 1.0 : 0.0;
                vd Dv = (tqq[i] * K.Sv_aa + tqr[i] * (K.Sv_ab * 2.0) + trr[i] * K.Sv_bb) * 0.5 + e3 * h;
                vd Dp = (tqq[i] * K.Sp_aa + tqr[i] * (K.Sp_ab * 2.0) + trr[i] * K.Sp_bb) * 0.5 + e3 * (0.5 * h2);
                W::st(lds, mb + (int(MB_PV) + (3 + i) * 8 + 7), Dv);
                W::st(lds, mb + (int(MB_PV) + i * 8 + 7), Dp);
                vd vn = x[3 + i] + Dv * c + acc[i] * h;
                vd pn = x[i] + x[3 + i] * h + Dp * c + acc[i] * (0.5 * h2);
                W::st(lds, mb + (int(MB_B) + 3 + i), vn - xn1[3 + i]);
                W::st(lds, mb + (int(MB_B) + i), pn - xn1[i]);
            }
            for (int i = 0; i < 4; ++i) W::st(lds, mb + (int(MB_B) + 6 + i), q[i] * K.A + r[i] * K.B - xn1[6 + i]);
        }
    }

    static NDP_D vd sg_lin(const RtiParams &P, const RkScal &K)
    {
        vd sg = (1.0 - K.a4) * P.two_over_h2;
        return sg * P.h4_12 - 0.5 * (P.dt * P.dt);
    }

    struct LamRegs { vd mm[9], own; };
    static NDP_D void lam_gather(const Tables &T, lp lds, vd h3, LamRegs &L)
    {
        W::st(lds, T.lam_w_off, h3);
        W::sync();
        for (int a = 0; a < 3; ++a) {
            L.mm[3 * a] = W::ld(lds, T.minor_one[a]);
            W::ld2(lds, T.minor_pair[a], L.mm[3 * a + 1], L.mm[3 * a + 2]);
        }
        L.own = W::ld(lds, T.own_off);
    }
    static NDP_D vd lam_cofactor(const Tables &T, const LamRegs &L)
    {
        const vd *mm = L.mm;
        vd d0 = mm[4] * mm[8] - mm[5] * mm[7];
        vd d1 = mm[3] * mm[8] - mm[5] * mm[6];
        vd d2 = mm[3] * mm[7] - mm[4] * mm[6];
        return (mm[0] * d0 - mm[1] * d1 + mm[2] * d2) * T.cof_sign;
    }
    static NDP_D vd lam_rdet(const Tables &T, const LamRegs &L, vd cof, bool &ok)
    {
        vd det = L.own * cof;
        det = det + W::csum1(det);
        det = det + W::csum2(det);
        vb pd = (det > 0.0) && (!T.lam_diag || (cof > 0.0));
        ok = W::all(pd) && ok;
        return W::rcp(det);
    }

    static NDP_D vd ldl_solve(const LdsMap &m, lp lds, vd rhs)
    {
        vi lane = W::lane_here();
        vi g = lane >> 4, j = W::lcol(lane);
        auto F = [&](int r, int c) { return W::ld(lds, lane * 0 + (m.SC + 4 * r + c)); };
        W::sync();
        W::st(lds, g * 16 + j + m.ZD, rhs);
        W::sync();
        const vd b0 = W::ld(lds, j + m.ZD), b1 = W::ld(lds, j + (m.ZD + 16)), b2 = W::ld(lds, j + (m.ZD + 32)), b3 = W::ld(lds, j + (m.ZD + 48));
        const vd l10 = F(1, 0), l20 = F(2, 0), l21 = F(2, 1), l30 = F(3, 0), l31 = F(3, 1), l32 = F(3, 2);
        const vd y0 = b0, y1 = b1 - l10 * y0, y2 = b2 - l20 * y0 - l21 * y1, y3 = b3 - l30 * y0 - l31 * y1 - l32 * y2;
        const vd x3 = y3 * F(3, 3);
        const vd x2 = y2 * F(2, 2) - l32 * x3;
        const vd x1 = y1 * F(1, 1) - l21 * x2 - l31 * x3;
        const vd x0 = y0 * F(0, 0) - l10 * x1 - l20 * x2 - l30 * x3;
        return W::sel(g == 0, x0, W::sel(g == 1, x1, W::sel(g == 2, x2, x3)));
    }
    static NDP_D void lam_factor_ldl(const LdsMap &m, const Tables &T, lp lds, vd h3, vb &okv)
    {
        W::st(lds, T.lam_w_off, h3);
        W::sync();
        auto A = [&](int r, int c) { return W::ld(lds, W::lane_here() * 0 + (m.SC + 4 * r + c)); };
        auto put = [&](int r, int c, vd v) { W::st(lds, W::lane_here() * 0 + (m.SC + 4 * r + c), v); };
        const vd d0 = A(0, 0), r0 = W::rcp(d0);
        const vd a10 = A(1, 0), a20 = A(2, 0), a30 = A(3, 0);
        const vd l10 = a10 * r0, l20 = a20 * r0, l30 = a30 * r0;
        const vd d1 = A(1, 1) - l10 * a10, r1 = W::rcp(d1);
        const vd l21 = (A(2, 1) - l20 * a10) * r1, l31 = (A(3, 1) - l30 * a10) * r1;
        const vd l21d = l21 * d1;
        const vd d2 = A(2, 2) - l20 * a20 - l21 * l21d, r2 = W::rcp(d2);
        const vd l32 = (A(3, 2) - l30 * a20 - l31 * l21d) * r2;
        const vd d3 = A(3, 3) - l30 * a30 - l31 * (l31 * d1) - l32 * (l32 * d2), r3 = W::rcp(d3);
        okv = okv && (d0 > 0.0) && (d1 > 0.0) && (d2 > 0.0) && (d3 > 0.0);
        W::sync();
        put(0, 0, r0); put(1, 1, r1); put(2, 2, r2); put(3, 3, r3);
        put(1, 0, l10); put(2, 0, l20); put(2, 1, l21); put(3, 0, l30); put(3, 1, l31); put(3, 2, l32);
        W::sync();
    }
    static NDP_D vd lam_inverse_ldl(const LdsMap &m, lp lds)
    {
        vi lane = W::lane_here();
        return ldl_solve(m, lds, W::sel((W::lcol(lane) & 3) == (lane >> 4), vd(1.0), vd(0.0)));
    }

    template <bool KEEP = false, bool ROBUST = false>
    static NDP_D bool riccati_sweep(const RtiParams &P, const LdsMap &m, const Tables &T, lp lds,
                                    const RtiIo *io = nullptr, md *linv = nullptr)
    {
        const int N = horizon(P);
        constexpr int UNROLL_SWEEP = ROBUST ? 1 : UNROLL_STAGES;
        (void)UNROLL_SWEEP;
        bool ok = true;
        vi lane = W::lane();
        vi g = lane >> 4, j = W::lcol(lane);
        vb okv = lane >= 0;
        md4 H;
        {
            md Pt[3];
            for (int c = 0; c < 3; ++c) Pt[c] = W::to_m(W::sel(j < 12, W::ld(lds, T.c_off[c] + cb(N)), vd(0.0)));
            md mk[3];
            for (int c = 0; c < 3; ++c) mk[c] = W::to_m(W::ld(lds, T.mk_off[c] + mb(N - 1)));
            for (int r = 0; r < 4; ++r) H.r[r] = W::to_m(W::ld(lds, T.c_off[r] + cb(N - 1)));
            md4 Wm = mman<3>(Pt, mk, W::mzero4());
            H = mman<3>(mk, Wm.r, H);
        }
        md mk[3], cc[4];
        {
            const int kn = N > 1 ? N - 2 : 0;
            for (int c = 0; c < 3; ++c) mk[c] = W::to_m(W::ld(lds, T.mk_off[c] + mb(kn)));
            for (int r = 0; r < 4; ++r) cc[r] = W::to_m(W::ld(lds, T.c_off[r] + cb(kn)));
        }
        md4 Ktp = W::mzero4();
        md Ktq = W::to_m(vd(0.0));
        int kprev = -1;
        NDP_UNROLL_SWEEP
        for (int k = N - 1; k >= 1; --k) {
            md nmk[3], ncc[4];
            const int kp = k >= 2 ? k - 2 : 0;
            md hux = H.r[3];
            if constexpr (ROBUST) {
                lam_factor_ldl(m, T, lds, W::to_d(hux), okv);
                if constexpr (KEEP) {
                    const vd inv = lam_inverse_ldl(m, lds);
                    linv_put(linv, k, N, W::to_m(MMA4 ? -inv : W::sel(T.kt_pred, -inv, vd(0.0))));
                }
                {
                    const vd G1 = ldl_solve(m, lds, W::to_d(hux));
                    vi ln = W::lane_here();
                    vi gg = ln >> 4, jj = W::lcol(ln);
                    W::st(lds, W::sel(jj < 12, jj * 4 + gg + m.KT, vi(m.MB + int(MB_DUMP))) + mb(k), -G1);
                }
                md rmk[3];
                for (int c = 0; c < 3; ++c) rmk[c] = W::to_m(W::ld(lds, T.mk_off[c] + mb(k - 1)));
                md4 Wf = mman<3>(H.r, rmk, W::mzero4());
                md4 Hb;
                for (int r = 0; r < 4; ++r) Hb.r[r] = W::to_m(W::ld(lds, T.c_off[r] + cb(k - 1)));
                Hb = mman<3>(rmk, Wf.r, Hb);
                md tt = Wf.r[3];
                const md G0 = W::to_m(ldl_solve(m, lds, W::to_d(tt)));
                md4 Hn = mma(-tt, G0, Hb);
                {
                    md ey[4];
                    vi ln = W::lane_here();
                    vi gg = ln >> 4, jj = W::lcol(ln);
                    for (int c = 0; c < 4; ++c) ey[c] = W::to_m(W::sel(jj == gg + 4 * c, vd(1.0), vd(0.0)));
                    md4 Tp = mman<4>(Hn.r, ey, W::mzero4());
                    for (int r = 0; r < 4; ++r) Hn.r[r] = W::mavg(Hn.r[r], Tp.r[r]);
                }
                H = Hn;
                continue;
            }
            NDP_FINE(const bool fst = io && io->dbg && k == N / 2; if (fst) fstamp(*io, m, 0, W::to_d(H.r[0]));)
            LamRegs LR;
            lam_gather(T, lds, W::to_d(hux), LR);
            NDP_FINE(if (fst) fstamp(*io, m, 1, LR.own);)
            md4 Wf = mman<3>(H.r, mk, W::mzero4());
            NDP_FINE(if (fst) fstamp(*io, m, 2, W::to_d(Wf.r[3]));)
            if (kprev >= 0) {
                if constexpr (MMA4) W::st(lds, T.kt_st4 + mb(kprev), W::to_d(Ktq));
                else for (int c = 0; c < 3; ++c) W::st(lds, T.kt_st[c] + mb(kprev), W::to_d(Ktp.r[c]));
            }
// ... 665 lines not shown
                        DeltaTabs DT;
                        build_delta_tabs(m, DT);
                        double corr = 0.0;
                        for (int rf = 0; rf < Q->refine; ++rf) {
                            refine_gradient(P, m, lds);
                            corr = delta_sweep<true>(P, m, T, DT, lds, linv);
                        }
                        if (pass && !(corr <= REFINE_FAIL)) ok = false;
                    }
                }
                NDP_FINE(if (fio && fio->dbg && iters == 1) fstamp(*fio, m, 7 + 3 * pass);)
                if (!ok) break;
                vd amin = 1.0;
                vd Ddtl[NSLOT], Ddtu[NSLOT], Ddll[NSLOT], Ddlu[NSLOT];
                for (int s = 0; s < NSLOT; ++s) {
                    vb v = S.valid[s];
                    vd zn = W::ld(lds, S.zoff[s]);
                    vd sl = pass ? vd(sigma_mu) - S.pl[s] : vd(0.0);
                    vd su = pass ? vd(sigma_mu) - S.pu[s] : vd(0.0);
                    vd lo, hi;
                    bounds(S, lds, s, lo, hi);
                    vd dtl = zn - lo - S.tl[s], dtu = hi - zn - S.tu[s];
                    vd rtl = W::rcp(S.tl[s]), rtu = W::rcp(S.tu[s]);
                    vd dll = sl * rtl - S.ll[s] - S.ll[s] * rtl * dtl;
                    vd dlu = su * rtu - S.lu[s] - S.lu[s] * rtu * dtu;
                    dtl = W::sel(v, dtl, vd(0.0)); dtu = W::sel(v, dtu, vd(0.0));
                    dll = W::sel(v, dll, vd(0.0)); dlu = W::sel(v, dlu, vd(0.0));
                    Ddtl[s] = dtl; Ddtu[s] = dtu; Ddll[s] = dll; Ddlu[s] = dlu;
                    amin = W::vmin(amin, W::sel(dtl < 0.0, -S.tl[s] * W::rcp(W::vmin(dtl, vd(-1e-300))), vd(1.0)));
                    amin = W::vmin(amin, W::sel(dtu < 0.0, -S.tu[s] * W::rcp(W::vmin(dtu, vd(-1e-300))), vd(1.0)));
                    amin = W::vmin(amin, W::sel(dll < 0.0, -S.ll[s] * W::rcp(W::vmin(dll, vd(-1e-300))), vd(1.0)));
                    amin = W::vmin(amin, W::sel(dlu < 0.0, -S.lu[s] * W::rcp(W::vmin(dlu, vd(-1e-300))), vd(1.0)));
                }
                double alpha = W::wave_min(amin);
                NDP_FINE(if (fio && fio->dbg && iters == 1) fstamp(*fio, m, 8 + 3 * pass);)
                if (pass == 0) {
                    vd acc = 0.0;
                    for (int s = 0; s < NSLOT; ++s) {
                        acc = acc + (S.ll[s] + Ddll[s] * alpha) * (S.tl[s] + Ddtl[s] * alpha)
                                  + (S.lu[s] + Ddlu[s] * alpha) * (S.tu[s] + Ddtu[s] * alpha);
                        S.pl[s] = Ddll[s] * Ddtl[s];
                        S.pu[s] = Ddlu[s] * Ddtu[s];
                    }
                    const double mu_aff = W::wave_sum(acc) * inv2m;
                    const double r = mu_aff / mu;
                    sigma_mu = fmax_u(r * r * r * mu, Q->mu_floor * Q->tol);
                } else {
                    if (alpha < 1.0) alpha *= Q->tau;
                    for (int t = 0; t < nzx + nzu; t += 64) {
                        vi i = lane + t;
                        vb p = i < nzx + nzu;
                        vd cur = W::ldp(lds, i + m.CX, p), nw = W::ldp(lds, i + m.ZX, p);
                        W::stp(lds, i + m.CX, cur + (nw - cur) * alpha, p);
                    }
                    vd acc = 0.0;
                    for (int s = 0; s < NSLOT; ++s) {
                        S.tl[s] = S.tl[s] + Ddtl[s] * alpha; S.tu[s] = S.tu[s] + Ddtu[s] * alpha;
                        S.ll[s] = S.ll[s] + Ddll[s] * alpha; S.lu[s] = S.lu[s] + Ddlu[s] * alpha;
                        acc = acc + S.ll[s] * S.tl[s] + S.lu[s] * S.tu[s];
                    }
                    mu = W::wave_sum(acc) * inv2m;
                    rho *= (1.0 - alpha);
                }
            }
            NDP_FINE(if (fio && fio->dbg && iters == 1) fstamp(*fio, m, 12);)
            if (!ok) { status = 4; failed = true; break; }
            if (!(mu == mu)) { status = 1; failed = true; break; }
        }
        iters_out += iters;
        return status;
    }

    static NDP_D double fmax_u(double a, double b) { return a > b ? a : b; }

    static NDP_D void fstamp(const RtiIo &io, const LdsMap &m, int idx, vd dep = vd(0.0))
    {
        vd t = W::clock_after(dep);
        W::gst(io.dbg, W::lane() * 0 + (m.total + 16 + idx), t, W::lane() == 0);
    }

    static NDP_D void stamp(const RtiIo &io, const LdsMap &m, int idx)
    {
        if (NDP_RARELY(io.dbg)) {
            vd t = W::clock();
            W::gst(io.dbg, W::lane() * 0 + (m.total + idx), t, W::lane() == 0);
        }
        if (NDP_RARELY(io.stamps)) {
            vd t = W::clock();
            W::gst(io.stamps, W::lane() * 0 + idx, t, W::lane() == 0);
        }
    }

    static NDP_D void issue_first(const RtiParams &P, const RtiIo &io, InBuf &inb, vd &x0v)
    {
        vi lane = W::lane();
        x0v = W::gldu(io.x0, W::imin(lane, NX - 1));
        RtiIo g = io;
        g.f_in_lds = 0;
        issue_inputs(P, g, inb, true);
    }

    static NDP_D void run(const RtiParams &P, const RtiIo &io, lp lds)
    {
        InBuf inb;
        vd x0v;
        issue_first(P, io, inb, x0v);
        run<false>(P, io, lds, inb, x0v);
    }


    template <bool DEFER, bool IPM_RARE = false, bool SENS = false, bool PSENS = false, bool VJP = false, bool WVJP = false, bool JVP = false>
    static NDP_D bool run(const RtiParams &P, const RtiIo &io, lp lds, InBuf &inb, vd x0v, const SensIo *sens = nullptr,
                          const PSensIo *psens = nullptr, const VjpIo *vjp = nullptr, double *gmodel = nullptr,
                          [[maybe_unused]] const JvpIo *jvp = nullptr)
    {
        const int N = horizon(P);
        const LdsMap m = make_map(N);
        const int nzx = (N + 1) * NX, nzu = N * NU;
        stamp(io, m, 0);
        vi lane = W::lane();
        int status = 0, iters = 0;
        typename W::late_t late_prev = W::late_none();
        vd fkeep[RF];
        for (int t = 0; t < RF; ++t) {
            vi i = lane + 64 * t;
            fkeep[t] = io.f_in_lds ? W::ldp(lds, i + m.TF, i < (N + 1) * 3) : vd(0.0);
        }
        Tables T;
        if (HT) load_tables(io.tables, T);
        else build_tables(m, T);
        stamp(io, m, 1);
        const int n_rti = NR ? NR : P.n_rti;
        const bool as_on = ASET && P.qp_mode == QP_AUTO && P.as_iter_max > 0;
        ActSet A;
        if (as_on) as_issue(P, io, A);
        else for (int t = 0; t < RUA; ++t) A.a[t] = vi(0);
        int sweeps = 0, cond_kept = 0;
        constexpr bool LOCAL_IN = NR >= 2;
        [[maybe_unused]] int zlast = m.ZX;
        for (int it = 0; it < n_rti; ++it) {
            InBuf lbuf;
            if constexpr (LOCAL_IN) {
                RtiIo g = io;
                g.f_in_lds = 0;
                x0v = W::gldu(io.x0, W::imin(lane_it(), NX - 1));
                issue_inputs(P, g, lbuf, it == 0);
            } else if (it > 0) issue_inputs(P, io, inb, false);
            InBuf &ib = LOCAL_IN ? lbuf : inb;
            if (io.f_in_lds)
                for (int t = 0; t < RF; ++t) ib.f[t] = fkeep[t];
            commit_inputs(P, m, ib, lds, it == 0, io);
            if (A_LDS && it == 0) { if (as_on) as_park(P, m, lds, A); else as_clear(P, m, lds, A); }
            stamp(io, m, 2);
            build_cost(P, m, lds);
            stamp(io, m, 3);
            vd fl[3] = {vd(0.0), vd(0.0), vd(0.0)};
            bool late_ok = true;
            if (io.f_late && P.use_fd) {
                vi k3 = W::imin(lane, N - 1) * 3;
                if (io.late_ready) {
                    for (int i = 0; i < 3; ++i) fl[i] = W::gldfu(io.f_late, k3 + i);
                } else if ((io.late_slow ? (W::count(io.late_slow), true) : true) &&
                           (late_ok = W::wait_ge(io.late_flag, io.late_flag2, io.late_want, io.late_timeout_us))) {
                    for (int i = 0; i < 3; ++i) fl[i] = W::gldf_fresh(io.f_late, k3 + i);
                } else if (io.late_missed) {
                    W::count(io.late_missed);
                }
            }
            linearize(P, m, lds);
            if (io.f_late && P.use_fd && late_ok) {
                W::sync();
                vi kk = W::imin(lane, N - 1);
                vi mb = kk * int(MB_STRIDE) + m.MB + int(MB_B);
                vb mine = lane < N;
                for (int i = 0; i < 3; ++i) {
                    vd a = fl[i] * P.inv_mass;
                    vd bp = W::ld(lds, mb + i), bv = W::ld(lds, mb + 3 + i);
                    W::stp(lds, mb + i, bp + a * (0.5 * P.dt * P.dt), mine);
                    W::stp(lds, mb + 3 + i, bv + a * P.dt, mine);
                }
            }
            if (!late_ok && !status) status = 5;
            if (io.f_late && it == 0) late_prev = W::late_count(io.late_cnt, io.late_group, io.late_group_size);
            stamp(io, m, 4);
            W::stp(lds, lane + m.ZX, x0v - W::ldp(lds, lane + m.XI, lane < NX), lane < NX);
            W::sync();
            if (NDP_RARELY(io.dbg && it == 0)) {
                for (int t = 0; t < m.total; t += 64) {
                    vi i = lane + t;
                    W::gst(io.dbg, i, W::ldp(lds, i, i < m.total), i < m.total);
                }
            }
            bool done = false, failed = false;
            bool pinned = false;
            int st = 0;
            if (DEFER || P.qp_mode == QP_AUTO) {
                if (NDP_RARELY(as_on && as_any(P, m, lds, A))) {
                    if (DEFER && A_LDS) return true;
                    as_apply(P, m, lds, A, pinned);
                }
                const int sweeps0 = sweeps;
                for (;;) {
                    stamp(io, m, 5);
                    bool ok = false, condensed = false;
                    if constexpr (COND != 0) {
                        if (!pinned && sweeps == sweeps0) {
                            condensed = W::template cond_solve<COND>(P, m, lds, N,
                                                                     [&](int r, int c) { return m_entry(m, r, c); }, [&](int r, int c) { return c_entry(m, r, c); });
                            condensed = condensed && cond_stationarity(P, m, lds) <= COND_STAT_MAX;
                            ok = condensed;
                        }
                    }
                    if (!condensed) ok = riccati_sweep(P, m, T, lds, &io);
                    stamp(io, m, 7);
                    ++sweeps;
                    if (NDP_RARELY(!ok)) {
                        if (!pinned) { st = 4; failed = true; done = true; }
                        break;
                    }
                    if (P.qp_mode != QP_AUTO) break;
                    const int verdict = as_check(P, m, lds, A, as_on, pinned);
                    if (verdict == 0) {
                        if (COND != 0 && condensed) cond_kept += COND_ACCEPTED;
                        done = true;
                        break;
                    }
                    if constexpr (COND != 0) {
                        if (condensed && verdict != 1) {
                            if (!pinned) as_save_b(P, m, lds);
                            pinned = true;
                            continue;
                        }
                    }
                    if (!DEFER && NDP_RARELY(as_on && verdict == 1 && sweeps - sweeps0 <= P.as_iter_max)) {
                        as_apply(P, m, lds, A, pinned);
                        continue;
                    }
                    break;
                }
            }
            const int zsrc = done ? m.ZX : m.CX;
            if constexpr (PSENS || VJP || JVP) zlast = zsrc;
            if (IPM_RARE ? NDP_RARELY(!done) : !done) {
                if (DEFER) return true;
                if (as_on) {
                    if (NDP_RARELY(pinned)) as_restore_b(P, m, lds);
                    as_clear(P, m, lds, A);
                    if (io.act) as_store(P, m, lds, io, A);
                }
                if constexpr (NSLOT <= 3) { if (io.ipm_ctr && it == 0) W::count64(io.ipm_ctr); }
                Slots S;
                build_slots(P, m, S);
                load_bounds(m, S, lds);
                st = ipm(P, m, T, S, lds, iters, failed, &io);
            }
            if (st && !status) status = st;
            {
                constexpr int RZ = RX + RU;
                const bool last = it + 1 == n_rti;
                const vi lane = lane_it();
                vd xa[RZ], xc[RZ];
                for (int t = 0; t < RZ; ++t) {
                    vi i = W::imin(lane + 64 * t, nzx + nzu - 1);
                    xa[t] = W::ld(lds, i + m.XI);
                    xc[t] = W::ld(lds, i + zsrc);
                }
                vb bad = lane < 0;
                for (int t = 0; t < RZ; ++t) bad = W::bor(bad, !(xc[t] == xc[t]));
                if (NDP_RARELY(!failed && W::any(bad))) {
                    failed = true;
                    if (!status) status = 1;
                }
                for (int t = 0; t < RZ; ++t) {
                    vi i = W::imin(lane + 64 * t, nzx + nzu - 1);
                    vd xn = failed ? xa[t] : xa[t] + xc[t];
                    if (!last) W::st(lds, i + m.XI, xn);
                    if (last) {
                        W::gst2(io.X, io.U, i, nzx, xn);
                        if (io.Xm) W::gst2(io.Xm, io.Um, i, nzx, xn);
                        if (t == (nzx >> 6)) {
                            vb pu = (i >= nzx) && (i < nzx + NU);
                            W::gst(io.u0, i - nzx, xn, pu);
                            if (NDP_RARELY(io.cmd != nullptr)) W::cmd_store(io.cmd, io.thrust_keep, io.kthr, io.cmd_mass, i - nzx, xn, pu);
                            if (W::any(pu && !(xn == xn))) status = 1;
                        }
                        if (nzx + NU > 64 * ((nzx >> 6) + 1) && t == (nzx >> 6) + 1) {
                            vb pu = (i >= nzx) && (i < nzx + NU);
                            W::gst(io.u0, i - nzx, xn, pu);
                            if (NDP_RARELY(io.cmd != nullptr)) W::cmd_store(io.cmd, io.thrust_keep, io.kthr, io.cmd_mass, i - nzx, xn, pu);
                            if (W::any(pu && !(xn == xn))) status = 1;
                        }
                    }
                }
            }
            W::sync();
        }
        stamp(io, m, 8);
        W::gsti(io.status, status);
        W::gsti(io.iters, iters + ((sweeps + cond_kept) << int(ITERS_SWEEP_SHIFT)));
        if (NDP_RARELY(as_on && io.act && sweeps != n_rti)) as_store(P, m, lds, io, A);
        if constexpr (SENS) {
            if (sens && sens->level > 0) sens_out(P, m, T, lds, A, status != 0, *sens);
        }
        if constexpr (PSENS) {
            if (psens) psens_out(P, m, lds, io, A, zlast, status != 0, *psens);
        }
        if constexpr (VJP) {
            if constexpr (WVJP) { if (vjp) vjp_out<true>(P, m, T, lds, io, A, zlast, status != 0, *vjp, gmodel); }
            else if (vjp) vjp_out(P, m, T, lds, io, A, zlast, status != 0, *vjp);
        }
        if constexpr (JVP) {
            if (jvp) jvp_out(P, m, T, lds, io, A, zlast, status != 0, *jvp);
        }
        if (io.f_late) W::late_publish(late_prev, io.late_gsize, io.late_done_word);
        return false;
    }

    static NDP_D void sens_out(const RtiParams &P, const LdsMap &m, const Tables &T, lp lds, const ActSet &A, bool bad, const SensIo &so)
    {
        const int N = horizon(P);
        vi lane = W::lane_here();
        for (int t = 0; t < RUA; ++t) {
// ... 477 lines not shown
```

Measured before the change: 46.10 million.

## Compute per-stage RK scalars once and share via LDS scratch in linearize

Linearization previously recomputed qdot and the RK scalars for every column task (4N + 3N + N lanes). Now each stage computes them once, one lane per stage, overlapped with build_cost. The results are stored to LDS scratch slots inside the unused K~' region, and the column tasks load them back. Constant factors are folded out of qdot and thrust_dir_tan, and column loads are issued one step ahead of their stores. The debug path is also extended to batches of up to 64, and register arrays are sized by the compile-time horizon. The cost is extra LDS traffic, an added sync, and higher register pressure from carrying StageLin across build_cost.

```diff
diff --git a/ndp_nmpc_qd_amd/batched.py b/ndp_nmpc_qd_amd/batched.py
--- a/ndp_nmpc_qd_amd/batched.py
+++ b/ndp_nmpc_qd_amd/batched.py
@@ -113,15 +113,16 @@
         return (u0, X, U, st, it) if full else u0
 
     def update_debug(self, x0, xr, ur, f=None, other=None, ego_xy=None):
-        x0, xr, ur = _lib.f64(x0, (1, 10)), _lib.f64(xr, (1, self.N + 1, 10)), _lib.f64(ur, (1, self.N, 4))
-        f32 = None if f is None else np.ascontiguousarray(f, dtype=np.float32).reshape(1, self.N + 1, 3)
-        other, ego_xy = _lib.f64(other, (1, self.N + 1, 10)), _lib.f64(ego_xy, (1, 2))
-        u0 = np.empty((1, 4))
-        dump = np.zeros(self._lib.ndp_debug_lds_doubles(self.N))
+        B = self.B
+        x0, xr, ur = _lib.f64(x0, (B, 10)), _lib.f64(xr, (B, self.N + 1, 10)), _lib.f64(ur, (B, self.N, 4))
+        f32 = None if f is None else np.ascontiguousarray(f, dtype=np.float32).reshape(B, self.N + 1, 3)
+        other, ego_xy = _lib.f64(other, (B, self.N + 1, 10)), _lib.f64(ego_xy, (B, 2))
+        u0 = np.empty((B, 4))
+        dump = np.zeros((B, self._lib.ndp_debug_lds_doubles(self.N)))
         self._check(self._lib.ndp_step_debug(self._h, _lib.ptr(x0), _lib.ptr(xr), _lib.ptr(ur), _lib.ptr(f32),
                                              _lib.ptr(other), _lib.ptr(ego_xy), _lib.ptr(u0), _lib.ptr(dump)),
                     "ndp_step_debug")
-        return u0, dump
+        return u0, (dump[0] if B == 1 else dump)
 
     def downwash(self, other, ego_ref, ego_xy=None):
         other = _lib.f64(other, (self.B, self.N + 1, 10))
diff --git a/ndp_nmpc_qd_amd/csrc/host.hpp b/ndp_nmpc_qd_amd/csrc/host.hpp
--- a/ndp_nmpc_qd_amd/csrc/host.hpp
+++ b/ndp_nmpc_qd_amd/csrc/host.hpp
@@ -70,6 +70,7 @@
     size_t off_x0 = 0, off_xr = 0, off_ur = 0, off_f = 0, off_other = 0, off_ego = 0, in_bytes = 0;
     size_t off_u0 = 0, off_st = 0, off_it = 0, out_bytes = 0, out_all = 0;
     double *sx0 = nullptr, *sxr = nullptr, *sur = nullptr, *sother = nullptr, *sego = nullptr, *su0 = nullptr, *sdbg = nullptr;
+    size_t sdbg_images = 0;
     float *sf = nullptr;
     int *dStatus = nullptr, *dIters = nullptr;
     const int *lastStatus = nullptr, *lastIters = nullptr;
diff --git a/ndp_nmpc_qd_amd/csrc/ndp_hip.hip b/ndp_nmpc_qd_amd/csrc/ndp_hip.hip
--- a/ndp_nmpc_qd_amd/csrc/ndp_hip.hip
+++ b/ndp_nmpc_qd_amd/csrc/ndp_hip.hip
@@ -330,6 +330,7 @@
         h->su0 = (double *)(h->dOut + h->off_u0); h->dStatus = (int *)(h->dOut + h->off_st); h->dIters = (int *)(h->dOut + h->off_it);
         h->lastStatus = h->dStatus; h->lastIters = h->dIters;
         ALLOC(h->sdbg, (size_t)(lds_doubles(cfg->N) + DBG_EXTRA) * 8);
+        h->sdbg_images = 1;
     }
 #undef ALLOC
     (void)hipMemsetAsync(h->dX, 0, nxs(h) * 8, h->stream);
@@ -614,6 +615,13 @@
     if (rc) return rc;
     if (h->slots_busy == 2) { h->err = "ndp_step_begin: two steps are already in flight (call ndp_step_end first)"; return -14; }
     if (h->ev_pending && (rc = wait_all(h))) return rc;
+    if (dump && h->sdbg_images < B) {
+        if ((rc = wait_all(h))) return rc;
+        (void)hipFree(h->sdbg);
+        h->sdbg = nullptr; h->sdbg_images = 0;
+        NDP_HIP(h, hipMalloc((void **)&h->sdbg, B * dbg_pitch(h->cfg.N) * 8));
+        h->sdbg_images = B;
+    }
     ndp_handle::HostSlot &sl = h->slot[h->slot_head];
     struct Seg { size_t off; const void *src; size_t len; size_t rows, row_len, src_stride; };
     Seg segs[6];
@@ -691,7 +699,7 @@
     for (int spin = 0; spin < 4000 && e == hipErrorNotReady; ++spin) e = hipEventQuery(sl.evOut);
     if (e == hipErrorNotReady) e = hipEventSynchronize(sl.evOut);
     if (e == hipSuccess && sl.dump)
-        e = hipMemcpy(sl.dump, h->sdbg, (size_t)(lds_doubles(h->cfg.N) + DBG_EXTRA) * 8, hipMemcpyDeviceToHost);
+        e = hipMemcpy(sl.dump, h->sdbg, B * dbg_pitch(h->cfg.N) * 8, hipMemcpyDeviceToHost);
     sl.busy = false;
     h->slot_tail ^= 1;
     --h->slots_busy;
@@ -790,7 +798,7 @@
 int ndp_step_debug(ndp_handle *h, const double *x0, const double *xr, const double *ur, const float *f,
                    const double *other, const double *ego_xy, double *u0, double *lds_dump)
 {
-    if (h && h->cfg.batch != 1) { h->err = "ndp_step_debug: batch must be 1"; return -9; }
+    if (h && h->cfg.batch > 64) { h->err = "ndp_step_debug: batch must be at most 64"; return -9; }
     return step_host(h, x0, xr, ur, f, other, ego_xy, u0, nullptr, nullptr, nullptr, nullptr, lds_dump);
 }
 
diff --git a/ndp_nmpc_qd_amd/csrc/rti_kernels.hip b/ndp_nmpc_qd_amd/csrc/rti_kernels.hip
--- a/ndp_nmpc_qd_amd/csrc/rti_kernels.hip
+++ b/ndp_nmpc_qd_amd/csrc/rti_kernels.hip
@@ -29,7 +29,7 @@
     io.u0 = bp.u0 + (size_t)inst * NU;
     io.status = bp.status + inst;
     io.iters = bp.iters + inst;
-    io.dbg = bp.dbg;
+    io.dbg = bp.dbg ? bp.dbg + (size_t)inst * dbg_pitch(N) : nullptr;
     io.f_in_lds = 0;
     io.kc = bp.kc;
     io.tables = bp.tables;
diff --git a/ndp_nmpc_qd_amd/csrc/rti_wave.hpp b/ndp_nmpc_qd_amd/csrc/rti_wave.hpp
--- a/ndp_nmpc_qd_amd/csrc/rti_wave.hpp
+++ b/ndp_nmpc_qd_amd/csrc/rti_wave.hpp
@@ -28,6 +28,8 @@
 enum { QP_AUTO = 0, QP_IPM_ALWAYS = 1 };
 enum { MB_STRIDE = 138, CB_STRIDE = 48 };
 enum { MB_PV = 0, MB_Q = 48, MB_B = 76, MB_ZERO = 86, MB_ONE = 87, MB_H = 88, MB_KT = 89, MB_DUMP = 137 };
+enum { LS_R = MB_KT + 1, LS_AB = LS_R + 4, LS_SV = LS_AB + 2, LS_Z = LS_SV + 8, LS_G = LS_Z + 16, LS_END = LS_G + 12 };
+static_assert(int(LS_END) <= int(MB_DUMP) && LS_R % 2 == 0 && MB_STRIDE % 2 == 0, "the scratch fits the K~' slots, pairs are 16-byte aligned");
 enum { CB_QQ = 0, CB_QE = 16, CB_RE = 26, CB_DEX = 30, CB_ZERO = 36, CB_QBV = 37, CB_DEU = 40, CB_RB = 44 };
 enum { KC_ZERO = 0, KC_ONE = 1, KC_H = 2, KC_QD = 3, KC_RD = 13, KC_LBV = 17, KC_UBV = 21, KC_LBU = 24, KC_UBU = 28, KC_SC = 32, KC_DUMP = 48,
        KC_LBVM = 50, KC_UBVM = 53, KC_LBUM = 56, KC_UBUM = 60, KC_SIZE = 64, KC_HOST = 64 };
@@ -150,6 +152,7 @@
 
 NDP_HD int lds_doubles(int N) { return make_map(N).total; }
 enum { DBG_EXTRA = 32 };
+NDP_HD size_t dbg_pitch(int N) { return (size_t)(lds_doubles(N) + DBG_EXTRA); }
 NDP_HD void lds_layout(int N, int *out)
 {
     const LdsMap m = make_map(N);
@@ -385,7 +388,9 @@
     }
 
     static constexpr int NMAXS = (64 * NSLOT + 3) / 7;
-    static constexpr int RX = ((NMAXS + 1) * NX + 63) / 64, RU = (NMAXS * NU + 63) / 64, RF = ((NMAXS + 1) * 3 + 63) / 64;
+    static constexpr int NH = NC > 0 ? NC : NMAXS;
+    static_assert(NC <= NMAXS, "the compile-time horizon needs more constraint slots");
+    static constexpr int RX = ((NH + 1) * NX + 63) / 64, RU = (NH * NU + 63) / 64, RF = ((NH + 1) * 3 + 63) / 64;
 
     struct InBuf { vd xr[RX], xi[RX], ur[RU], ui[RU], f[RF], kc; };
 
@@ -440,11 +445,12 @@
         W::sync();
     }
 
-    static NDP_D void build_cost(const RtiParams &P, const LdsMap &m, lp lds)
+    struct StageLin;
+    static NDP_D void build_cost(const RtiParams &P, const LdsMap &m, lp lds, StageLin &S)
     {
         const int N = horizon(P);
         vi lane = lane_it();
-        constexpr int RA = (4 * (NMAXS + 1) + 63) / 64, RB = (6 * (NMAXS + 1) + 63) / 64, RC = (4 * NMAXS + 63) / 64;
+        constexpr int RA = (4 * (NH + 1) + 63) / 64, RB = (6 * (NH + 1) + 63) / 64, RC = (4 * NH + 63) / 64;
         vd qr[RA][4], qi[RA][4];
         vd xb[RB], rb[RB], wb[RB], uc[RC], rc[RC], wc[RC];
         for (int t = 0; t < RA; ++t) {
@@ -469,6 +475,8 @@
             uc[t] = W::ld(lds, ti + m.UI);
             rc[t] = W::ld(lds, ti + m.TUR);
         }
+        stage_issue(P, m, lds, S);
+        stage_head(P, lds, S);
         for (int t = 0; t < RA; ++t) {
             vi task = W::imin(lane + 64 * t, 4 * (N + 1) - 1);
             vi k = task >> 2;
@@ -517,12 +525,12 @@
         }
     }
 
-    static NDP_D void qdot(const vd q[4], const vd w[3], vd o[4])
-    {
-        o[0] = (-w[0] * q[1] - w[1] * q[2] - w[2] * q[3]) * 0.5;
-        o[1] = (w[0] * q[0] + w[2] * q[2] - w[1] * q[3]) * 0.5;
-        o[2] = (w[1] * q[0] - w[2] * q[1] + w[0] * q[3]) * 0.5;
-        o[3] = (w[2] * q[0] + w[1] * q[1] - w[0] * q[2]) * 0.5;
+    static NDP_D void qdot(const vd q[4], const vd wh[3], vd o[4])
+    {
+        o[0] = -wh[0] * q[1] - wh[1] * q[2] - wh[2] * q[3];
+        o[1] = wh[0] * q[0] + wh[2] * q[2] - wh[1] * q[3];
+        o[2] = wh[1] * q[0] - wh[2] * q[1] + wh[0] * q[3];
+        o[3] = wh[2] * q[0] + wh[1] * q[1] - wh[0] * q[2];
     }
     static NDP_D void thrust_dir(const vd q[4], vd o[3])
     {
@@ -532,9 +540,9 @@
     }
     static NDP_D void thrust_dir_tan(const vd q[4], const vd s[4], vd o[3])
     {
-        o[0] = (s[1] * q[3] + q[1] * s[3] + s[0] * q[2] + q[0] * s[2]) * 2.0;
-        o[1] = (s[2] * q[3] + q[2] * s[3] - s[0] * q[1] - q[0] * s[1]) * 2.0;
-        o[2] = (q[1] * s[1] + q[2] * s[2]) * -4.0;
+        o[0] = s[1] * q[3] + q[1] * s[3] + s[0] * q[2] + q[0] * s[2];
+        o[1] = s[2] * q[3] + q[2] * s[3] - s[0] * q[1] - q[0] * s[1];
+        o[2] = q[1] * s[1] + q[2] * s[2];
     }
 
     struct RkScal {
@@ -557,113 +565,180 @@
         K.Sp_bb = (2.0 * hh * hh) * hp;
     }
 
-    static NDP_D void linearize(const RtiParams &P, const LdsMap &m, lp lds)
+    struct StageLin { vd x[10], xn1[10], w[3], c, f[3], r[4]; RkScal K; vi mb; };
+    static_assert(NMAXS <= 64, "one lane per stage: one round");
+
+    static NDP_D void stage_issue(const RtiParams &P, const LdsMap &m, lp lds, StageLin &S)
     {
         const int N = horizon(P);
+        vi k = W::imin(lane_it(), N - 1);
+        S.mb = k * int(MB_STRIDE) + m.MB;
+        vi xi = k * NX + m.XI, ui = k * NU + m.UI, fi = k * 3 + m.TF;
+        for (int i = 0; i < 10; ++i) S.x[i] = W::ld(lds, xi + i);
+        for (int i = 0; i < 3; ++i) S.w[i] = W::ld(lds, ui + i);
+        S.c = W::ld(lds, ui + 3);
+        for (int i = 0; i < 3; ++i) S.f[i] = W::ld(lds, fi + i);
+        for (int i = 0; i < 10; ++i) S.xn1[i] = W::ld(lds, xi + (NX + i));
+    }
+
+    static NDP_D void stage_head(const RtiParams &P, lp lds, StageLin &S)
+    {
+        const vd *q = S.x + 6;
+        const vd wh[3] = {S.w[0] * 0.5, S.w[1] * 0.5, S.w[2] * 0.5}, qh[4] = {q[0] * 0.5, q[1] * 0.5, q[2] * 0.5, q[3] * 0.5};
+        qdot(q, wh, S.r);
+        RkScal &K = S.K;
+        rk_scalars(P, wh[0] * wh[0] + wh[1] * wh[1] + wh[2] * wh[2], K);
+        const vi mb = S.mb;
+        const vd sc[LS_Z - LS_R] = {S.r[0], S.r[1], S.r[2], S.r[3], K.A, K.B, K.Sv_aa, K.Sv_ab, K.Sv_bb, K.Sp_aa, K.Sp_ab, K.a3, K.a4, K.b4};
+        for (int i = 0; i < LS_Z - LS_R; ++i) W::st(lds, mb + (int(LS_R) + i), sc[i]);
+        const vd o = vd(0.0);
+        const vd Z[16] = {o, -wh[0], -wh[1], -wh[2],  wh[0], o, wh[2], -wh[1],  wh[1], -wh[2], o, wh[0],  wh[2], wh[1], -wh[0], o};
+        for (int i = 0; i < 16; ++i) W::st(lds, mb + (int(LS_Z) + i), Z[i]);
+        const vd G[12] = {-qh[1], -qh[2], -qh[3],  qh[0], -qh[3], qh[2],  qh[3], qh[0], -qh[1],  -qh[2], qh[1], qh[0]};
+        for (int i = 0; i < 12; ++i) W::st(lds, mb + (int(LS_G) + i), G[i]);
+        W::st(lds, mb + int(MB_ZERO), vd(0.0));
+        W::st(lds, mb + int(MB_ONE), vd(1.0));
+        W::st(lds, mb + int(MB_H), vd(P.dt));
+    }
+
+    static NDP_D void stage_tail(const RtiParams &P, lp lds, const StageLin &S)
+    {
+        const double h = P.dt, h2 = h * h;
+        const vd *x = S.x, *xn1 = S.xn1, *q = S.x + 6, *r = S.r;
+        const RkScal &K = S.K;
+        const vd c = S.c;
+        const vi mb = S.mb;
+        const vd acc[3] = {S.f[0] * P.inv_mass, S.f[1] * P.inv_mass, S.f[2] * P.inv_mass - P.g};
+        vd tqq[3], tqr[3], trr[3];
+        thrust_dir_tan(q, q, tqq); thrust_dir_tan(q, r, tqr); thrust_dir_tan(r, r, trr);
+        for (int i = 0; i < 3; ++i) {
+            vd Dv = tqq[i] * K.Sv_aa + tqr[i] * (K.Sv_ab * 2.0) + trr[i] * K.Sv_bb;
+            vd Dp = tqq[i] * K.Sp_aa + tqr[i] * (K.Sp_ab * 2.0) + trr[i] * K.Sp_bb;
+            if (i == 2) { Dv = Dv * -2.0 + h; Dp = Dp * -2.0 + 0.5 * h2; }
+            else { Dv = Dv + 0.0 * h; Dp = Dp + 0.0 * (0.5 * h2); }
+            W::st(lds, mb + (int(MB_PV) + (3 + i) * 8 + 7), Dv);
+            W::st(lds, mb + (int(MB_PV) + i * 8 + 7), Dp);
+            vd vn = x[3 + i] + Dv * c + acc[i] * h;
+            vd pn = x[i] + x[3 + i] * h + Dp * c + acc[i] * (0.5 * h2);
+            W::st(lds, mb + (int(MB_B) + 3 + i), vn - xn1[3 + i]);
+            W::st(lds, mb + (int(MB_B) + i), pn - xn1[i]);
+        }
+        for (int i = 0; i < 4; ++i) W::st(lds, mb + (int(MB_B) + 6 + i), q[i] * K.A + r[i] * K.B - xn1[6 + i]);
+    }
+
+    struct ColQ { vd q[4], c, r[4], A, B, Sv_aa, Sv_ab, Sv_bb, Sp_aa, Sp_ab, z[4]; vi mb, j; };
+    struct ColW { vd q[4], c, eps, r[4], B, Sv_ab, Sv_bb, Sp_ab, a3, a4, b4, g[4]; vi mb; };
+    static constexpr int RQ = (4 * NH + 63) / 64, RW = (3 * NH + 63) / 64;
+    static constexpr bool COLS_AHEAD = NSLOT <= 3;
+
+    static NDP_D void colq_load(const LdsMap &m, lp lds, int N, vi lane, int t, ColQ &C)
+    {
+        vi task = W::imin(lane + 64 * t, 4 * N - 1);
+        vi k = task >> 2;
+        C.j = task & 3;
+        vi xi = k * NX + (m.XI + 6), ui = k * NU + m.UI, ls = k * int(MB_STRIDE) + m.MB;
+        for (int i = 0; i < 4; ++i) C.q[i] = W::ld(lds, xi + i);
+        C.c = W::ld(lds, ui + 3);
+        W::ld2(lds, ls + int(LS_R), C.r[0], C.r[1]); W::ld2(lds, ls + (int(LS_R) + 2), C.r[2], C.r[3]);
+        W::ld2(lds, ls + int(LS_AB), C.A, C.B);
+        W::ld2(lds, ls + int(LS_SV), C.Sv_aa, C.Sv_ab); W::ld2(lds, ls + (int(LS_SV) + 2), C.Sv_bb, C.Sp_aa);
+        C.Sp_ab = W::ld(lds, ls + (int(LS_SV) + 4));
+        C.mb = ls + C.j;
+        for (int i = 0; i < 4; ++i) C.z[i] = W::ld(lds, C.mb + (int(LS_Z) + 4 * i));
+    }
+    static NDP_D void colq_store(lp lds, const ColQ &C, vd Sp_bb)
+    {
+        const vd *q = C.q, *r = C.r, *z = C.z;
+        vd e[4], Uv[4], Vv[4], Up[4], Vp[4], t1[3], t2[3];
+        for (int i = 0; i < 4; ++i) e[i] = W::sel(C.j == i, vd(1.0), vd(0.0));
+        for (int i = 0; i < 4; ++i) {
+            Uv[i] = e[i] * C.Sv_aa + z[i] * C.Sv_ab; Vv[i] = e[i] * C.Sv_ab + z[i] * C.Sv_bb;
+            Up[i] = e[i] * C.Sp_aa + z[i] * C.Sp_ab; Vp[i] = e[i] * C.Sp_ab + z[i] * Sp_bb;
+        }
+        const vd c2 = C.c * 2.0, c4 = C.c * -4.0;
+        const vi mb = C.mb;
+        thrust_dir_tan(q, Uv, t1); thrust_dir_tan(r, Vv, t2);
+        for (int i = 0; i < 3; ++i) W::st(lds, mb + (int(MB_PV) + (3 + i) * 8), (t1[i] + t2[i]) * (i == 2 ? c4 : c2));
+        thrust_dir_tan(q, Up, t1); thrust_dir_tan(r, Vp, t2);
+        for (int i = 0; i < 3; ++i) W::st(lds, mb + (int(MB_PV) + i * 8), (t1[i] + t2[i]) * (i == 2 ? c4 : c2));
+        for (int i = 0; i < 4; ++i) W::st(lds, mb + (int(MB_Q) + i * 7), e[i] * C.A + z[i] * C.B);
+    }
+    static NDP_D void colw_load(const LdsMap &m, lp lds, int N, vi lane, int t, ColW &C)
+    {
+        vi task = W::imin(lane + 64 * t, 3 * N - 1);
+        vi k = W::div3(task);
+        vi mm = task - k * 3;
+        vi xi = k * NX + (m.XI + 6), ui = k * NU + m.UI, ls = k * int(MB_STRIDE) + m.MB;
+        for (int i = 0; i < 4; ++i) C.q[i] = W::ld(lds, xi + i);
+        C.c = W::ld(lds, ui + 3);
+        C.eps = W::ld(lds, ui + mm);
+        W::ld2(lds, ls + int(LS_R), C.r[0], C.r[1]); W::ld2(lds, ls + (int(LS_R) + 2), C.r[2], C.r[3]);
+        C.B = W::ld(lds, ls + (int(LS_AB) + 1));
+        C.Sv_ab = W::ld(lds, ls + (int(LS_SV) + 1)); C.Sv_bb = W::ld(lds, ls + (int(LS_SV) + 2));
+        W::ld2(lds, ls + (int(LS_SV) + 4), C.Sp_ab, C.a3); W::ld2(lds, ls + (int(LS_SV) + 6), C.a4, C.b4);
+        C.mb = ls + 4 + mm;
+        for (int i = 0; i < 4; ++i) C.g[i] = W::ld(lds, ls + mm + (int(LS_G) + 3 * i));
+    }
+    static NDP_D void colw_store(const RtiParams &P, lp lds, const ColW &C, vd Sp_bb)
+    {
         const double h = P.dt, h2 = h * h, hh = 0.5 * h, h6 = P.h_6, hp = P.h2_6;
+        const vd *q = C.q, *r = C.r, *g = C.g;
+        const vd eps = C.eps * 0.5, a3 = C.a3, a4 = C.a4, b4 = C.b4;
+        const double da3 = -0.25 * h2, da4 = -0.5 * h2, db4 = -0.25 * h * h2;
+        vd Sv_aad = (a3 * (2.0 * da3) + a4 * da4) * h6, Sv_abd = (a4 * db4) * h6;
+        vd Sv_bad = (b4 * da4 + 2.0 * hh * da3) * h6, Sv_bbd = (b4 * db4) * h6;
+        vd Sp_aad = a3 * (da3 * hp);
+        const double Sp_bad = hh * da3 * hp;
+        vd dA = sg_lin(P, a4), dB = vd(-P.h3_6);
+        vd Uv[4], Vv[4], Up[4], Vp[4], t1[3], t2[3];
+        for (int i = 0; i < 4; ++i) {
+            Uv[i] = (q[i] * Sv_aad + r[i] * Sv_abd) * eps + g[i] * C.Sv_ab;
+            Vv[i] = (q[i] * Sv_bad + r[i] * Sv_bbd) * eps + g[i] * C.Sv_bb;
+            Up[i] = (q[i] * Sp_aad) * eps + g[i] * C.Sp_ab;
+            Vp[i] = (q[i] * Sp_bad) * eps + g[i] * Sp_bb;
+        }
+        const vi mb = C.mb;
+        const vd c2 = C.c * 2.0, c4 = C.c * -4.0;
+        thrust_dir_tan(q, Uv, t1); thrust_dir_tan(r, Vv, t2);
+        for (int i = 0; i < 3; ++i) W::st(lds, mb + (int(MB_PV) + (3 + i) * 8), (t1[i] + t2[i]) * (i == 2 ? c4 : c2));
+        thrust_dir_tan(q, Up, t1); thrust_dir_tan(r, Vp, t2);
+        for (int i = 0; i < 3; ++i) W::st(lds, mb + (int(MB_PV) + i * 8), (t1[i] + t2[i]) * (i == 2 ? c4 : c2));
+        for (int i = 0; i < 4; ++i) W::st(lds, mb + (int(MB_Q) + i * 7), (q[i] * dA + r[i] * dB) * eps + g[i] * C.B);
+    }
+
+    static NDP_D void linearize(const RtiParams &P, const LdsMap &m, lp lds, const StageLin &S)
+    {
+        const int N = horizon(P);
+        const double hh = 0.5 * P.dt, hp = P.h2_6;
+        const vd Sp_bb = vd((2.0 * hh * hh) * hp);
         vi lane = lane_it();
-        for (int t = 0; t < 4 * N; t += 64) {
-            vi task = W::imin(lane + t, 4 * N - 1);
-            vi k = task >> 2;
-            vi j = task & 3;
-            vi xi = k * NX + m.XI + 6, ui = k * NU + m.UI;
-            vd q[4] = {W::ld(lds, xi), W::ld(lds, xi + 1), W::ld(lds, xi + 2), W::ld(lds, xi + 3)};
-            vd w[3] = {W::ld(lds, ui), W::ld(lds, ui + 1), W::ld(lds, ui + 2)};
-            vd c = W::ld(lds, ui + 3);
-            vd r[4], e[4], z[4];
-            qdot(q, w, r);
-            RkScal K;
-            rk_scalars(P, (w[0] * w[0] + w[1] * w[1] + w[2] * w[2]) * 0.25, K);
-            for (int i = 0; i < 4; ++i) e[i] = W::sel(j == i, vd(1.0), vd(0.0));
-            qdot(e, w, z);
-            vd Uv[4], Vv[4], Up[4], Vp[4], t1[3], t2[3];
-            for (int i = 0; i < 4; ++i) {
-                Uv[i] = e[i] * K.Sv_aa + z[i] * K.Sv_ab; Vv[i] = e[i] * K.Sv_ab + z[i] * K.Sv_bb;
-                Up[i] = e[i] * K.Sp_aa + z[i] * K.Sp_ab; Vp[i] = e[i] * K.Sp_ab + z[i] * K.Sp_bb;
-            }
-            vi mb = k * int(MB_STRIDE) + m.MB + j;
-            thrust_dir_tan(q, Uv, t1); thrust_dir_tan(r, Vv, t2);
-            for (int i = 0; i < 3; ++i) W::st(lds, mb + (int(MB_PV) + (3 + i) * 8), (t1[i] + t2[i]) * c);
-            thrust_dir_tan(q, Up, t1); thrust_dir_tan(r, Vp, t2);
-            for (int i = 0; i < 3; ++i) W::st(lds, mb + (int(MB_PV) + i * 8), (t1[i] + t2[i]) * c);
-            for (int i = 0; i < 4; ++i) W::st(lds, mb + (int(MB_Q) + i * 7), e[i] * K.A + z[i] * K.B);
-        }
-        for (int t = 0; t < 3 * N; t += 64) {
-            vi task = W::imin(lane + t, 3 * N - 1);
-            vi k = W::div3(task);
-            vi mm = task - k * 3;
-            vi xi = k * NX + m.XI + 6, ui = k * NU + m.UI;
-            vd q[4] = {W::ld(lds, xi), W::ld(lds, xi + 1), W::ld(lds, xi + 2), W::ld(lds, xi + 3)};
-            vd w[3] = {W::ld(lds, ui), W::ld(lds, ui + 1), W::ld(lds, ui + 2)};
-            vd c = W::ld(lds, ui + 3);
-            vd r[4], em[3], g[4];
-            qdot(q, w, r);
-            RkScal K;
-            rk_scalars(P, (w[0] * w[0] + w[1] * w[1] + w[2] * w[2]) * 0.25, K);
-            for (int i = 0; i < 3; ++i) em[i] = W::sel(mm == i, vd(1.0), vd(0.0));
-            qdot(q, em, g);
-            vd eps = (em[0] * w[0] + em[1] * w[1] + em[2] * w[2]) * 0.5;
-            const double da3 = -0.25 * h2, da4 = -0.5 * h2, db4 = -0.25 * h * h2;
-            vd Sv_aad = (K.a3 * (2.0 * da3) + K.a4 * da4) * h6, Sv_abd = (K.a4 * db4) * h6;
-            vd Sv_bad = (K.b4 * da4 + 2.0 * hh * da3) * h6, Sv_bbd = (K.b4 * db4) * h6;
-            vd Sp_aad = K.a3 * (da3 * hp);
-            const double Sp_bad = hh * da3 * hp;
-            vd dA = sg_lin(P, K), dB = vd(-P.h3_6);
-            vd Uv[4], Vv[4], Up[4], Vp[4], t1[3], t2[3];
-            for (int i = 0; i < 4; ++i) {
-                Uv[i] = (q[i] * Sv_aad + r[i] * Sv_abd) * eps + g[i] * K.Sv_ab;
-                Vv[i] = (q[i] * Sv_bad + r[i] * Sv_bbd) * eps + g[i] * K.Sv_bb;
-                Up[i] = (q[i] * Sp_aad) * eps + g[i] * K.Sp_ab;
-                Vp[i] = (q[i] * Sp_bad) * eps + g[i] * K.Sp_bb;
-            }
-            vi mb = k * int(MB_STRIDE) + m.MB + 4 + mm;
-            thrust_dir_tan(q, Uv, t1); thrust_dir_tan(r, Vv, t2);
-            for (int i = 0; i < 3; ++i) W::st(lds, mb + (int(MB_PV) + (3 + i) * 8), (t1[i] + t2[i]) * c);
-            thrust_dir_tan(q, Up, t1); thrust_dir_tan(r, Vp, t2);
-            for (int i = 0; i < 3; ++i) W::st(lds, mb + (int(MB_PV) + i * 8), (t1[i] + t2[i]) * c);
-            for (int i = 0; i < 4; ++i) W::st(lds, mb + (int(MB_Q) + i * 7), (q[i] * dA + r[i] * dB) * eps + g[i] * K.B);
-        }
-        for (int t = 0; t < N; t += 64) {
-            vi k = W::imin(lane + t, N - 1);
-            {
-                vi mc = k * int(MB_STRIDE) + m.MB;
-                W::st(lds, mc + int(MB_ZERO), vd(0.0));
-                W::st(lds, mc + int(MB_ONE), vd(1.0));
-                W::st(lds, mc + int(MB_H), vd(P.dt));
-            }
-            vi xi = k * NX + m.XI, ui = k * NU + m.UI, fi = k * 3 + m.TF;
-            vd x[10];
-            for (int i = 0; i < 10; ++i) x[i] = W::ld(lds, xi + i);
-            vd w[3] = {W::ld(lds, ui), W::ld(lds, ui + 1), W::ld(lds, ui + 2)};
-            vd c = W::ld(lds, ui + 3);
-            vd acc[3] = {W::ld(lds, fi) * P.inv_mass, W::ld(lds, fi + 1) * P.inv_mass, W::ld(lds, fi + 2) * P.inv_mass - P.g};
-            vd xn1[10];
-            for (int i = 0; i < 10; ++i) xn1[i] = W::ld(lds, xi + (NX + i));
-            vd q[4] = {x[6], x[7], x[8], x[9]}, r[4];
-            qdot(q, w, r);
-            RkScal K;
-            rk_scalars(P, (w[0] * w[0] + w[1] * w[1] + w[2] * w[2]) * 0.25, K);
-            vd tqq[3], tqr[3], trr[3];
-            thrust_dir_tan(q, q, tqq); thrust_dir_tan(q, r, tqr); thrust_dir_tan(r, r, trr);
-            vi mb = k * int(MB_STRIDE) + m.MB;
-            for (int i = 0; i < 3; ++i) {
-                const double e3 = i == 2 ? 1.0 : 0.0;
-                vd Dv = (tqq[i] * K.Sv_aa + tqr[i] * (K.Sv_ab * 2.0) + trr[i] * K.Sv_bb) * 0.5 + e3 * h;
-                vd Dp = (tqq[i] * K.Sp_aa + tqr[i] * (K.Sp_ab * 2.0) + trr[i] * K.Sp_bb) * 0.5 + e3 * (0.5 * h2);
-                W::st(lds, mb + (int(MB_PV) + (3 + i) * 8 + 7), Dv);
-                W::st(lds, mb + (int(MB_PV) + i * 8 + 7), Dp);
-                vd vn = x[3 + i] + Dv * c + acc[i] * h;
-                vd pn = x[i] + x[3 + i] * h + Dp * c + acc[i] * (0.5 * h2);
-                W::st(lds, mb + (int(MB_B) + 3 + i), vn - xn1[3 + i]);
-                W::st(lds, mb + (int(MB_B) + i), pn - xn1[i]);
-            }
-            for (int i = 0; i < 4; ++i) W::st(lds, mb + (int(MB_B) + 6 + i), q[i] * K.A + r[i] * K.B - xn1[6 + i]);
-        }
-    }
-
-    static NDP_D vd sg_lin(const RtiParams &P, const RkScal &K)
-    {
-        vd sg = (1.0 - K.a4) * P.two_over_h2;
+        W::sync();
+        if constexpr (COLS_AHEAD) {
+            ColQ cq[RQ];
+            ColW cw[RW];
+            bool issued[RQ + RW] = {};
+            colq_load(m, lds, N, lane, 0, cq[0]);
+            issued[0] = true;
+            stage_tail(P, lds, S);
+            for (int i = 0; i < RQ + RW; ++i) {
+                for (int n = i; n <= i + 1 && n < RQ + RW; ++n) {
+                    if (issued[n] || !(n < RQ ? 64 * n < 4 * N : 64 * (n - RQ) < 3 * N)) continue;
+                    if (n < RQ) colq_load(m, lds, N, lane, n, cq[n]); else colw_load(m, lds, N, lane, n - RQ, cw[n - RQ]);
+                    issued[n] = true;
+                }
+                if (!issued[i]) continue;
+                if (i < RQ) colq_store(lds, cq[i], Sp_bb); else colw_store(P, lds, cw[i - RQ], Sp_bb);
+            }
+        } else {
+            stage_tail(P, lds, S);
+            for (int t = 0; t < RQ; ++t) if (64 * t < 4 * N) { ColQ c; colq_load(m, lds, N, lane, t, c); colq_store(lds, c, Sp_bb); }
+            for (int t = 0; t < RW; ++t) if (64 * t < 3 * N) { ColW c; colw_load(m, lds, N, lane, t, c); colw_store(P, lds, c, Sp_bb); }
+        }
+    }
+
+    static NDP_D vd sg_lin(const RtiParams &P, vd a4)
+    {
+        vd sg = (1.0 - a4) * P.two_over_h2;
         return sg * P.h4_12 - 0.5 * (P.dt * P.dt);
     }
 
@@ -1635,7 +1710,8 @@
             commit_inputs(P, m, ib, lds, it == 0, io);
             if (A_LDS && it == 0) { if (as_on) as_park(P, m, lds, A); else as_clear(P, m, lds, A); }
             stamp(io, m, 2);
-            build_cost(P, m, lds);
+            StageLin sl;
+            build_cost(P, m, lds, sl);
             stamp(io, m, 3);
             vd fl[3] = {vd(0.0), vd(0.0), vd(0.0)};
             bool late_ok = true;
@@ -1650,7 +1726,7 @@
                     W::count(io.late_missed);
                 }
             }
-            linearize(P, m, lds);
+            linearize(P, m, lds, sl);
             if (io.f_late && P.use_fd && late_ok) {
                 W::sync();
                 vi kk = W::imin(lane, N - 1);
```

Result: no change. 46.31 million, median of 3 (+0.5%).
